# szcompressor/SZ3

Measured on AMD Instinct MI355X. Metric: compression throughput GB/s + ratio at fixed abs errBound, 512^3 f32, higher is better.
Workload: dtype f32; 1 GPU; C2: 3D float32 512x512x512 synthetic field per GPU, Lorenzo predictor, abs errBound=0.001, device-resident in -> device-resident Huffman payload; parallelism=slab1, algo=HIP_LORENZO(16), exchange=none (one rank)

## Files before the change

include/sz3hip.h:

```cpp
#ifndef SZ3HIP_H
#define SZ3HIP_H
#include <stddef.h>
#include <stdint.h>

#ifdef __cplusplus
extern "C" {
#endif

#define SZ3HIP_FLOAT 0
#define SZ3HIP_DOUBLE 1
#define SZ3HIP_UINT8 2
#define SZ3HIP_INT8 3
#define SZ3HIP_UINT16 4
#define SZ3HIP_INT16 5
#define SZ3HIP_UINT32 6
#define SZ3HIP_INT32 7
#define SZ3HIP_UINT64 8
#define SZ3HIP_INT64 9

enum { SZ3HIP_EB_ABS = 0, SZ3HIP_EB_REL, SZ3HIP_EB_PSNR, SZ3HIP_EB_L2NORM, SZ3HIP_EB_ABS_AND_REL, SZ3HIP_EB_ABS_OR_REL };

enum {
    SZ3HIP_ALGO_LORENZO_REG = 0,
    SZ3HIP_ALGO_INTERP_LORENZO = 1,
// ... 51 lines not shown
size_t sz3hip_compress_blob(sz3hip_config *conf, int dataType, const void *data, char *blob, size_t cap);
int sz3hip_decompress_blob(const sz3hip_config *conf, int dataType, const char *blob, size_t size, void *decData);
int sz3hip_peek_config(sz3hip_config *conf, const char *cmpData, size_t cmpSize);

typedef struct sz3hip_ctx sz3hip_ctx;

sz3hip_ctx *sz3hip_ctx_create(int device, uint64_t max_elems, int dataType);
void sz3hip_ctx_destroy(sz3hip_ctx *ctx);
size_t sz3hip_payload_bound(const sz3hip_ctx *ctx, uint64_t n);
size_t sz3hip_payload_bound_max(const sz3hip_ctx *ctx, uint64_t n);
size_t sz3hip_payload_bound_conf(const sz3hip_ctx *ctx, const sz3hip_config *conf, int worst_case);

int sz3hip_minmax_device(sz3hip_ctx *ctx, const void *d_in, uint64_t n, double *min_out, double *max_out, void *stream);

int sz3hip_compress_stage1(sz3hip_ctx *ctx, const sz3hip_config *conf, const void *d_in, void *stream);
void *sz3hip_histogram_ptr(sz3hip_ctx *ctx);
size_t sz3hip_histogram_len(const sz3hip_ctx *ctx);
int sz3hip_ctx_set_histogram(sz3hip_ctx *ctx, void *d_hist);
int sz3hip_compress_stage2(sz3hip_ctx *ctx, void *d_payload, size_t cap, void *stream);
int sz3hip_compress_finish(sz3hip_ctx *ctx, size_t *payload_size, void *stream);
int sz3hip_compress_device(sz3hip_ctx *ctx, const sz3hip_config *conf, const void *d_in, void *d_payload, size_t cap,
                           size_t *payload_size, void *stream);
int sz3hip_decompress_device(sz3hip_ctx *ctx, const void *d_payload, size_t payload_size, void *d_out, void *stream);

typedef struct sz3hip_stats {
    uint64_t n, n_value_outliers, n_delta_outliers, n_chunks, bitstream_bytes, payload_bytes;
    uint32_t n_symbols, max_code_len;
    uint32_t narrow_codes;
    uint32_t reserved;
} sz3hip_stats;
int sz3hip_get_stats(sz3hip_ctx *ctx, sz3hip_stats *st);

typedef struct sz3hip_tuner_report {
    int32_t ran;
    int32_t use_interp;
    uint64_t sample_block_size, n_filtered, n_blocks;
    int32_t profiling;
    int32_t interpAlgo, interpDirection;
    int32_t speculated;
    double interpAlpha, interpBeta;
    double est_bytes[8];
} sz3hip_tuner_report;
int sz3hip_get_tuner_report(sz3hip_ctx *ctx, sz3hip_tuner_report *rep);

void sz3hip_set_profiling(sz3hip_ctx *ctx, int on);
int sz3hip_get_stage_times(sz3hip_ctx *ctx, const char **names, float *ms, int max);
void sz3hip_ctx_forget(sz3hip_ctx *ctx);
void sz3hip_ctx_set_speculation(sz3hip_ctx *ctx, int off);
void sz3hip_ctx_set_deterministic(sz3hip_ctx *ctx, int on);
void sz3hip_ctx_set_tuner_exact(sz3hip_ctx *ctx, int on);
void sz3hip_get_spec_stats(const sz3hip_ctx *ctx, uint32_t *hits, uint32_t *misses);
int sz3hip_last_call_fused(const sz3hip_ctx *ctx);
int sz3hip_last_call_q16(const sz3hip_ctx *ctx);
void sz3hip_ctx_set_fused(sz3hip_ctx *ctx, int on);
int sz3hip_lab_build(void);
int sz3hip_debug_copy_codes(sz3hip_ctx *ctx, uint16_t *host_codes, uint64_t n);
int sz3hip_debug_decode_info(sz3hip_ctx *ctx, uint32_t *out4);
void sz3hip_debug_force_generic(int on);
void sz3hip_debug_flags(int flags);

typedef struct sz3hip_comm sz3hip_comm;
#define SZ3HIP_COMM_ID_BYTES 128
sz3hip_comm *sz3hip_comm_create_local(int ndev, const int *devices);
int sz3hip_comm_unique_id(unsigned char *id128);
sz3hip_comm *sz3hip_comm_create_rank(int nranks, int rank, int device, const unsigned char *id128);
void sz3hip_comm_destroy(sz3hip_comm *comm);
int sz3hip_comm_size(const sz3hip_comm *comm);
int sz3hip_comm_rank(const sz3hip_comm *comm);
int sz3hip_comm_local_size(const sz3hip_comm *comm);
int sz3hip_comm_device(const sz3hip_comm *comm, int member);
int sz3hip_comm_allreduce_histogram(sz3hip_comm *comm, sz3hip_ctx *const *ctxs, void *const *streams);
int sz3hip_comm_allreduce_u64(sz3hip_comm *comm, void *const *d_bufs, size_t count, void *const *streams);
int sz3hip_comm_allreduce_minmax(sz3hip_comm *comm, double *mins, double *maxs, void *const *streams);


size_t sz3hip_compress_rank(sz3hip_comm *comm, const sz3hip_config *global_conf, int dataType, const void *slab_data,
                            char *blob, size_t cap, sz3hip_config *slab_conf);
size_t sz3hip_assemble_container(const sz3hip_config *global_conf, int dataType, int G, const sz3hip_config *slab_confs,
                                 const char *const *blobs, const size_t *blob_sizes, char *out, size_t cap);

#ifdef __cplusplus
}
#endif
#endif
```

sz3_amd/__init__.py:

```python
import ctypes as C
import os

import numpy as np

_HERE = os.path.dirname(os.path.abspath(__file__))
LIB_PATH = os.environ.get("SZ3HIP_LIB") or os.path.join(_HERE, "libsz3hip.so")

EB_ABS, EB_REL, EB_PSNR, EB_L2NORM, EB_ABS_AND_REL, EB_ABS_OR_REL = range(6)
ALGO_LORENZO_REG, ALGO_INTERP_LORENZO, ALGO_INTERP, ALGO_NOPRED, ALGO_LOSSLESS = range(5)
ALGO_HIP_LORENZO = 16
ALGO_HIP_INTERP = 17
INTERP_ALGO_LINEAR, INTERP_ALGO_CUBIC = 0, 1
SZ_FLOAT, SZ_DOUBLE = 0, 1


class SZ3HipError(RuntimeError):
    def __init__(self, code, msg):
        super().__init__("sz3hip error %d: %s" % (code, msg))
        self.code = code


class _CConfig(C.Structure):
    _fields_ = [
        ("N", C.c_int32), ("dims", C.c_uint64 * 4), ("num", C.c_uint64),
        ("cmprAlgo", C.c_uint8), ("errorBoundMode", C.c_uint8),
        ("absErrorBound", C.c_double), ("relErrorBound", C.c_double),
        ("psnrErrorBound", C.c_double), ("l2normErrorBound", C.c_double),
        ("openmp", C.c_uint8), ("quantbinCnt", C.c_int32), ("blockSize", C.c_int32),
        ("predDim", C.c_uint8), ("dataType", C.c_uint8),
        ("lorenzo", C.c_uint8), ("lorenzo2", C.c_uint8), ("regression", C.c_uint8), ("regression2", C.c_uint8),
        ("interpAlgo", C.c_uint8), ("interpDirection", C.c_uint8),
        ("interpAnchorStride", C.c_int32), ("interpAlpha", C.c_double), ("interpBeta", C.c_double),
    ]


class _CTunerReport(C.Structure):
    _fields_ = [("ran", C.c_int32), ("use_interp", C.c_int32), ("sample_block_size", C.c_uint64), ("n_filtered", C.c_uint64),
                ("n_blocks", C.c_uint64), ("profiling", C.c_int32), ("interpAlgo", C.c_int32), ("interpDirection", C.c_int32),
                ("speculated", C.c_int32), ("interpAlpha", C.c_double), ("interpBeta", C.c_double), ("est_bytes", C.c_double * 8)]


class _CStats(C.Structure):
    _fields_ = [("n", C.c_uint64), ("n_value_outliers", C.c_uint64), ("n_delta_outliers", C.c_uint64),
                ("n_chunks", C.c_uint64), ("bitstream_bytes", C.c_uint64), ("payload_bytes", C.c_uint64),
                ("n_symbols", C.c_uint32), ("max_code_len", C.c_uint32),
                ("narrow_codes", C.c_uint32), ("reserved", C.c_uint32)]


_lib = None


def _share_torch_hip_runtime():
    try:
        import importlib.util
        import sys
        if "torch" in sys.modules:
            return
        if os.environ.get("SZ3HIP_TORCH_PRELOAD", "0") == "1":
# ... 56 lines not shown
    L.sz3hip_compress.argtypes = [P(_CConfig), C.c_int, C.c_void_p, C.c_void_p, C.c_size_t]
    L.sz3hip_decompress.restype = C.c_int
    L.sz3hip_decompress.argtypes = [P(_CConfig), C.c_int, C.c_void_p, C.c_size_t, C.c_void_p]
    L.sz3hip_peek_config.restype = C.c_int
    L.sz3hip_compress_from_device.restype = C.c_size_t
    L.sz3hip_compress_from_device.argtypes = [P(_CConfig), C.c_int, C.c_void_p, P(C.c_int64), C.c_void_p, C.c_size_t, C.c_void_p]
    L.sz3hip_decompress_to_device.restype = C.c_int
    L.sz3hip_decompress_to_device.argtypes = [P(_CConfig), C.c_int, C.c_void_p, C.c_size_t, C.c_void_p, P(C.c_int64), C.c_void_p]
    L.sz3hip_peek_config.argtypes = [P(_CConfig), C.c_void_p, C.c_size_t]
    L.sz3hip_ctx_create.restype = C.c_void_p
    L.sz3hip_ctx_create.argtypes = [C.c_int, C.c_uint64, C.c_int]
    L.sz3hip_ctx_destroy.argtypes = [C.c_void_p]
    L.sz3hip_payload_bound.restype = C.c_size_t
    L.sz3hip_payload_bound.argtypes = [C.c_void_p, C.c_uint64]
    L.sz3hip_payload_bound_max.restype = C.c_size_t
    L.sz3hip_payload_bound_max.argtypes = [C.c_void_p, C.c_uint64]
    L.sz3hip_minmax_device.restype = C.c_int
    L.sz3hip_minmax_device.argtypes = [C.c_void_p, C.c_void_p, C.c_uint64, P(C.c_double), P(C.c_double), C.c_void_p]
    L.sz3hip_compress_stage1.restype = C.c_int
    L.sz3hip_compress_stage1.argtypes = [C.c_void_p, P(_CConfig), C.c_void_p, C.c_void_p]
    L.sz3hip_histogram_ptr.restype = C.c_void_p
    L.sz3hip_histogram_ptr.argtypes = [C.c_void_p]
    L.sz3hip_histogram_len.restype = C.c_size_t
    L.sz3hip_histogram_len.argtypes = [C.c_void_p]
    L.sz3hip_ctx_set_histogram.restype = C.c_int
    L.sz3hip_ctx_set_histogram.argtypes = [C.c_void_p, C.c_void_p]
    L.sz3hip_compress_stage2.restype = C.c_int
    L.sz3hip_compress_stage2.argtypes = [C.c_void_p, C.c_void_p, C.c_size_t, C.c_void_p]
    L.sz3hip_compress_finish.restype = C.c_int
    L.sz3hip_compress_finish.argtypes = [C.c_void_p, P(C.c_size_t), C.c_void_p]
    L.sz3hip_compress_device.restype = C.c_int
    L.sz3hip_compress_device.argtypes = [C.c_void_p, P(_CConfig), C.c_void_p, C.c_void_p, C.c_size_t, P(C.c_size_t), C.c_void_p]
    L.sz3hip_decompress_device.restype = C.c_int
    L.sz3hip_decompress_device.argtypes = [C.c_void_p, C.c_void_p, C.c_size_t, C.c_void_p, C.c_void_p]
    L.sz3hip_get_stats.restype = C.c_int
    L.sz3hip_get_stats.argtypes = [C.c_void_p, P(_CStats)]
    L.sz3hip_get_tuner_report.restype = C.c_int
    L.sz3hip_get_tuner_report.argtypes = [C.c_void_p, P(_CTunerReport)]
    L.sz3hip_set_profiling.argtypes = [C.c_void_p, C.c_int]
    L.sz3hip_ctx_forget.argtypes = [C.c_void_p]
    L.sz3hip_ctx_forget.restype = None
    L.sz3hip_ctx_set_speculation.argtypes = [C.c_void_p, C.c_int]
    L.sz3hip_ctx_set_speculation.restype = None
    L.sz3hip_ctx_set_deterministic.argtypes = [C.c_void_p, C.c_int]
    L.sz3hip_ctx_set_deterministic.restype = None
    L.sz3hip_ctx_set_tuner_exact.argtypes = [C.c_void_p, C.c_int]
    L.sz3hip_ctx_set_tuner_exact.restype = None
    L.sz3hip_set_stock_format.argtypes = [C.c_int]
    L.sz3hip_set_stock_format.restype = None
    L.sz3hip_last_call_fused.argtypes = [C.c_void_p]
    L.sz3hip_last_call_fused.restype = C.c_int
    L.sz3hip_last_call_q16.argtypes = [C.c_void_p]
    L.sz3hip_last_call_q16.restype = C.c_int
    L.sz3hip_ctx_set_fused.argtypes = [C.c_void_p, C.c_int]
    L.sz3hip_ctx_set_fused.restype = None
    L.sz3hip_get_spec_stats.argtypes = [C.c_void_p, C.POINTER(C.c_uint32), C.POINTER(C.c_uint32)]
    L.sz3hip_get_spec_stats.restype = None
    L.sz3hip_payload_bound_conf.restype = C.c_size_t
    L.sz3hip_payload_bound_conf.argtypes = [C.c_void_p, C.c_void_p, C.c_int]
    L.sz3hip_get_stage_times.restype = C.c_int
    L.sz3hip_get_stage_times.argtypes = [C.c_void_p, P(C.c_char_p), P(C.c_float), C.c_int]
    L.sz3hip_debug_copy_codes.restype = C.c_int
    L.sz3hip_debug_copy_codes.argtypes = [C.c_void_p, C.c_void_p, C.c_uint64]
    L.sz3hip_debug_force_generic.argtypes = [C.c_int]
    L.sz3hip_config_load_n.restype = C.c_size_t
    L.sz3hip_config_load_n.argtypes = [P(_CConfig), C.c_void_p, C.c_size_t]
    L.sz3hip_comm_create_local.restype = C.c_void_p
    L.sz3hip_comm_create_local.argtypes = [C.c_int, P(C.c_int)]
    L.sz3hip_comm_unique_id.restype = C.c_int
    L.sz3hip_comm_unique_id.argtypes = [C.c_void_p]
    L.sz3hip_comm_create_rank.restype = C.c_void_p
    L.sz3hip_comm_create_rank.argtypes = [C.c_int, C.c_int, C.c_int, C.c_void_p]
    L.sz3hip_comm_destroy.argtypes = [C.c_void_p]
    for f in ("size", "rank", "local_size"):
        getattr(L, "sz3hip_comm_" + f).restype = C.c_int
        getattr(L, "sz3hip_comm_" + f).argtypes = [C.c_void_p]
    L.sz3hip_comm_device.restype = C.c_int
    L.sz3hip_comm_device.argtypes = [C.c_void_p, C.c_int]
    L.sz3hip_comm_allreduce_histogram.restype = C.c_int
    L.sz3hip_comm_allreduce_histogram.argtypes = [C.c_void_p, P(C.c_void_p), P(C.c_void_p)]
    L.sz3hip_comm_allreduce_u64.restype = C.c_int
    L.sz3hip_comm_allreduce_u64.argtypes = [C.c_void_p, P(C.c_void_p), C.c_size_t, P(C.c_void_p)]
    L.sz3hip_comm_allreduce_minmax.restype = C.c_int
    L.sz3hip_comm_allreduce_minmax.argtypes = [C.c_void_p, P(C.c_double), P(C.c_double), P(C.c_void_p)]
    L.sz3hip_compress_rank.restype = C.c_size_t
    L.sz3hip_compress_rank.argtypes = [C.c_void_p, P(_CConfig), C.c_int, C.c_void_p, C.c_void_p, C.c_size_t, P(_CConfig)]
    L.sz3hip_assemble_container.restype = C.c_size_t
    L.sz3hip_assemble_container.argtypes = [P(_CConfig), C.c_int, C.c_int, P(_CConfig), P(C.c_void_p), P(C.c_size_t), C.c_void_p, C.c_size_t]
    L.SZ_compress_args.restype = C.c_void_p
    L.SZ_compress_args.argtypes = [C.c_int, C.c_void_p, P(C.c_size_t), C.c_int, C.c_double, C.c_double, C.c_double,
                                   C.c_size_t, C.c_size_t, C.c_size_t, C.c_size_t, C.c_size_t]
    L.SZ_decompress.restype = C.c_void_p
    L.SZ_decompress.argtypes = [C.c_int, C.c_void_p, C.c_size_t, C.c_size_t, C.c_size_t, C.c_size_t, C.c_size_t, C.c_size_t]
    L.free_buf.argtypes = [C.c_void_p]
    _lib = L
    return L


def _check(rc):
    if rc != 0:
        raise SZ3HipError(rc, lib().sz3hip_last_error().decode())


_SZ_TYPES = {"float32": 0, "float64": 1, "uint8": 2, "int8": 3, "uint16": 4, "int16": 5, "uint32": 6, "int32": 7, "uint64": 8, "int64": 9}


# ... 221 lines not shown

    def finish(self, stream=0):
        sz = C.c_size_t()
        _check(lib().sz3hip_compress_finish(self._h, C.byref(sz), stream))
        return int(sz.value)

    def compress(self, conf, d_in, d_payload, cap, stream=0):
        sz = C.c_size_t()
        _check(lib().sz3hip_compress_device(self._h, C.byref(conf._c), d_in, d_payload, int(cap), C.byref(sz), stream))
        return int(sz.value)

    def decompress(self, d_payload, size, d_out, stream=0):
        _check(lib().sz3hip_decompress_device(self._h, d_payload, int(size), d_out, stream))

    def stats(self):
        st = _CStats()
        lib().sz3hip_get_stats(self._h, C.byref(st))
        return {k: int(getattr(st, k)) for k, _ in _CStats._fields_}

    def tuner_report(self):
        r = _CTunerReport()
        lib().sz3hip_get_tuner_report(self._h, C.byref(r))
        out = {k: getattr(r, k) for k, _ in _CTunerReport._fields_ if k not in ("est_bytes", "speculated")}
        out["est_bytes"] = [float(x) for x in r.est_bytes]
        self.speculated = int(r.speculated)
        return out

    def set_profiling(self, on=True):
        lib().sz3hip_set_profiling(self._h, int(on))

    def forget(self):
        lib().sz3hip_ctx_forget(self._h)

    def set_speculation(self, on=True, backoff=True):
        lib().sz3hip_ctx_set_speculation(self._h, (0 if backoff else 2) if on else 1)

    def set_deterministic(self, on=True):
        lib().sz3hip_ctx_set_deterministic(self._h, int(on))

    def set_tuner_exact(self, on=True):
        lib().sz3hip_ctx_set_tuner_exact(self._h, int(on))

    def set_fused(self, on=True):
        lib().sz3hip_ctx_set_fused(self._h, int(on))

    @property
    def fused(self):
        return bool(lib().sz3hip_last_call_fused(self._h))

    @property
    def q16(self):
        return bool(lib().sz3hip_last_call_q16(self._h))

    def spec_stats(self):
        h, m = C.c_uint32(), C.c_uint32()
        lib().sz3hip_get_spec_stats(self._h, C.byref(h), C.byref(m))
        return int(h.value), int(m.value)

    def payload_bound_conf(self, conf, worst_case=False):
        return int(lib().sz3hip_payload_bound_conf(self._h, C.byref(conf._c), int(bool(worst_case))))

    def stage_times(self):
        names = (C.c_char_p * 16)()
        ms = (C.c_float * 16)()
        k = lib().sz3hip_get_stage_times(self._h, names, ms, 16)
        return {names[i].decode(): float(ms[i]) for i in range(k)}

    def debug_codes(self, n):
        out = np.empty(int(n), dtype=np.uint16)
        _check(lib().sz3hip_debug_copy_codes(self._h, out.ctypes.data, int(n)))
        return out


COMM_ID_BYTES = 128


class Comm:

    def __init__(self, handle):
        if not handle:
            raise SZ3HipError(lib().sz3hip_last_error_code(), lib().sz3hip_last_error().decode())
        self._h = handle

    @staticmethod
    def unique_id():
        buf = (C.c_ubyte * COMM_ID_BYTES)()
        _check(lib().sz3hip_comm_unique_id(buf))
        return bytes(buf)

    @classmethod
    def local(cls, ndev=0, devices=None):
        arr = (C.c_int * len(devices))(*devices) if devices else None
        return cls(lib().sz3hip_comm_create_local(int(ndev if not devices else len(devices)), arr))

    @classmethod
    def rank(cls, nranks, rank, device, id_bytes):
        b = (C.c_ubyte * COMM_ID_BYTES).from_buffer_copy(bytes(id_bytes))
        return cls(lib().sz3hip_comm_create_rank(int(nranks), int(rank), int(device), b))

    def close(self):
        if self._h:
            lib().sz3hip_comm_destroy(self._h)
            self._h = None

    @property
    def size(self):
# ... 60 lines not shown
```

sz3_amd/csrc/sz3hip_api.cpp:

```cpp
#include <hip/hip_runtime.h>

#include <dlfcn.h>
#include <math.h>
#include <stdarg.h>
#include <stdio.h>
#include <stdlib.h>
#include <string.h>

#include <sched.h>
#include <unistd.h>
#include <algorithm>
#include <atomic>
#include <chrono>
#include <mutex>
#include <string>
#include <thread>
#include <vector>

#include "../../include/sz3c.h"
#include "../../include/sz3hip.h"
#include "sz3hip_format.h"
#include "sz3hip_internal.h"
#include "sz3hip_stock_geom.h"
#include "sz3hip_kernels.h"
// ... 504 lines not shown
    hh.eb = eb;
    hh.n = num;
    hh.chunk_syms = SZH_CHUNK_SYMS;
    hh.n_chunks = (num + SZH_CHUNK_SYMS - 1) / SZH_CHUNK_SYMS;
    hh.interp_alpha = ip.alpha;
    hh.interp_beta = ip.beta;
    hh.interp_id = (uint32_t)ip.interp_id;
    hh.interp_dir = (uint32_t)ip.direction;
    hh.anchor_stride = ip.anchor_stride;
    ctx->stage1_done = true;
    ctx->stage2_done = false;
    return 0;
}

static bool book_spec_ok(const sz3hip_ctx *ctx, uint32_t predictor, uint32_t radius) {
    return ctx->book_idx >= 0 && ctx->spec_off != 1 && (ctx->spec_skip == 0 || ctx->spec_off == 2) && !(szk_dbg_flags & 131072) &&
           ctx->book_pred == predictor && ctx->book_radius == radius;
}
static int lorenzo_k1(sz3hip_ctx *ctx, int N, const uint64_t *dims, const void *d_in, double eb, int radius, uint64_t num,
                      uint64_t out_cap, bool allow_narrow, szk_k1_params &p, hipStream_t s) {
    memset(&p, 0, sizeof(p));
    for (int i = 0; i < 4; i++) p.d[i] = 1;
    for (int i = 0; i < N; i++) p.d[4 - N + i] = dims[i];
    p.lat = szk_make_lattice(eb);
    p.radius = (uint32_t)radius;
    p.out_cap = out_cap;
    p.hist = ctx->d_hist;
    p.hist_partial = ctx->d_hist_partial;
    p.n_vout = ctx->d_counters + 0;
    p.n_dout = ctx->d_counters + 1;
    p.vout_idx = ctx->d_vout_idx;
    p.dout_idx = ctx->d_dout_idx;
    p.vout_val = ctx->d_vout_val;
    p.dout_val = ctx->d_dout_val;
    p.mode.probe_big = reinterpret_cast<uint32_t *>(ctx->d_counters + 4);
    p.mode.n_total = num;
    p.mode.n_samples = (num / SZK_PROBE_STRIDE) * 64 + std::min<uint64_t>(64, num % SZK_PROBE_STRIDE);
    p.mode.allow = allow_narrow && radius >= 128;
    p.mode.pack_wide = allow_narrow ? (uint32_t)ctx->pack_wide : 0u;
    p.wide16 = ctx->wide16 < 0 ? (ctx->dtype == SZ3HIP_DOUBLE ? 1u : 0u) : (uint32_t)ctx->wide16;
    p.range = reinterpret_cast<uint32_t *>(ctx->d_counters + 8);
    p.hint_narrow = allow_narrow ? ctx->narrow_hint : -1;
    if ((ctx->hist_exposed || ctx->hist_reduced) && p.hint_narrow > 0) p.hint_narrow = -1;
    p.hint_q16 = allow_narrow && ctx->dtype == SZ3HIP_FLOAT && ctx->q16_hint > 0 && ctx->q16_block == 0 ? 1 : 0;
    p.q16_flag = reinterpret_cast<uint32_t *>(ctx->d_counters + 11) + 1;
    const bool samp = allow_narrow && radius >= 128 && N <= 3 && p.d[3] % 256 == 0 && num >= SZK_SAMP_MIN_ELEMS && !ctx->hist_exposed && !ctx->hist_reduced &&
                      !(szk_dbg_flags & 65536);
    if (samp) {
        const int fresh = ctx->book_idx < 0 ? 0 : 1 - ctx->book_idx;
        p.samp.words = reinterpret_cast<uint32_t *>(ctx->d_counters + 16);
        p.samp.enc = ctx->bk[fresh].enc;
        p.samp.lens = ctx->bk[fresh].lens;
        p.samp.info = ctx->bk[fresh].info;
        p.seg_bits = ctx->d_seg_bits;
        p.seg_made = reinterpret_cast<uint32_t *>(ctx->d_counters + 10) + 1;
    }
    if (!samp && allow_narrow && book_spec_ok(ctx, 0, (uint32_t)radius) && ctx->cb_hint == 0 && !ctx->lists_long && !ctx->hist_exposed) {
        p.spec_lens = ctx->bk[ctx->book_idx].lens;
        p.seg_bits = ctx->d_seg_bits;
        p.seg_made = reinterpret_cast<uint32_t *>(ctx->d_counters + 10) + 1;
        p.defer_fold = ctx->hist_exposed || ctx->hist_reduced || (szk_dbg_flags & 16777216) ? 0 : 1;
        const uint64_t need = szk_fuse_scratch_words(N, p.d);
        if (need && ctx->fuse_on && !ctx->hist_reduced && (!ctx->spec_exact || ctx->last_spec_hit)) {
            p.fuse_slots = reinterpret_cast<uint32_t *>(ctx->d_codes);
            p.fuse_cap_words = (ctx->max_n + 64) / 2;
            if (need > p.fuse_cap_words && need <= 2 * num + (1u << 18)) {
                if (ctx->fuse_scratch_words < need) {
                    if (ctx->d_fuse_scratch) (void)hipFree(ctx->d_fuse_scratch);
                    ctx->d_fuse_scratch = nullptr;
                    ctx->fuse_scratch_words = 0;
                    if (hipMalloc((void **)&ctx->d_fuse_scratch, need * 4) == hipSuccess) ctx->fuse_scratch_words = need;
                    else (void)hipGetLastError();
                }
                if (ctx->fuse_scratch_words >= need) {
                    p.fuse_slots = ctx->d_fuse_scratch;
                    p.fuse_cap_words = ctx->fuse_scratch_words;
                }
            }
            p.fuse = 1;
            p.fuse_enc = ctx->bk[ctx->book_idx].enc;
            p.fuse_info = ctx->bk[ctx->book_idx].info;
            p.seg_base = ctx->d_seg_base;
            p.fuse_flag = reinterpret_cast<uint32_t *>(ctx->d_counters + 11);
        }
    }
    p.prof_ev0 = p.prof_ev1 = nullptr;
    if (ctx->profiling && allow_narrow) {
        p.prof_ev0 = ctx->ev[ST_K1_KERNEL][0];
        p.prof_ev1 = ctx->ev[ST_K1_KERNEL][1];
        ctx->ev_used[ST_K1_KERNEL] = true;
    }
    return szk_launch_k1(ctx->dtype, N, d_in, ctx->d_codes, &p, s);
}
static int stage1_lorenzo(sz3hip_ctx *ctx, const sz3hip_config *conf, const void *d_in, double eb, int radius, uint64_t num, hipStream_t s) {
    szk_k1_params p;
    prof_begin(ctx, ST_K1, s);
    int rc = lorenzo_k1(ctx, conf->N, conf->dims, d_in, eb, radius, num, ctx->cur_out_cap, true, p, s);
    ctx->mode = p.mode;
    ctx->range_ready = p.range_kept != 0;
    ctx->s1_assumed_narrow = p.assumed_narrow != 0;
    ctx->s1_q16 = p.assumed_q16 != 0;
    ctx->s1_spec = p.spec_lens != nullptr;
    ctx->seg_expected = p.seg_expected != 0 && !(szk_dbg_flags & 33554432);
    ctx->fold_rows = p.defer_fold ? p.fold_rows : 0;
    ctx->fold_range = p.range;
    ctx->s1_fused = p.fused != 0;
// ... 1003 lines not shown
        if (ctx->range_ready && !cb.range_ready)
            HIPCHK(hipMemsetAsync(ctx->d_counters + 8, 0, 16, s));
        prof_begin(ctx, ST_CODEBOOK, s);
        int rcb = szk_launch_codebook(ctx->d_hist, &cb, s);
        prof_end(ctx, ST_CODEBOOK, s);
        if (rcb) return fail(SZ3HIP_EHIP, "codebook kernel launch failed (%d)", rcb);
    }
    szk_layout_params lp;
    lp.proto = ctx->proto;
    lp.n_vout = ctx->d_counters + 0;
    lp.n_dout = ctx->d_counters + 1;
    lp.out_cap = ctx->cur_out_cap;
    lp.info = ctx->bk[used].info;
    lp.state = ctx->d_state;
    lp.side_bytes = ctx->proto.predictor == 2 ? ctx->d_blk_counters + 2 : nullptr;
    szk_asm_params ap;
    memset(&ap, 0, sizeof(ap));
    ap.n_vout = ctx->d_counters + 0;
    ap.n_dout = ctx->d_counters + 1;
    ap.out_cap = ctx->cur_out_cap;
    ap.t_is_32bit = ap.q_is_32bit = ctx->dtype == SZ3HIP_FLOAT;
    ap.state = ctx->d_state;
    ap.payload = (uint8_t *)d_payload;
    ap.cap = cap;
    ap.total_words = ctx->d_counters + 2;
    ap.lens = ctx->bk[used].lens;
    ap.chunk_words = ctx->d_chunk_words;
    ap.sub_bits = ctx->d_sub_bits;
    ap.vout_idx = ctx->d_vout_idx;
    ap.dout_idx = ctx->d_dout_idx;
    ap.vout_val = ctx->d_vout_val;
    ap.dout_val = ctx->d_dout_val;
    ap.side = ctx->proto.predictor == 2 ? ctx->d_blk_side : nullptr;
    ap.assumed_narrow = ctx->s1_assumed_narrow ? 1 : 0;
    ap.q16_flag = ctx->s1_q16 && ctx->proto.predictor == 0 ? reinterpret_cast<const uint32_t *>(ctx->d_counters + 11) + 1 : nullptr;
    ap.mode = ctx->mode;
    ap.samp_words = samp_words;
    szk_merge_args mg;
    memset(&mg, 0, sizeof(mg));
    const bool merge = fused && ctx->s1_fused && ctx->seg_expected;
    if (ctx->s1_fused && !merge) return fail(SZ3HIP_EHIP, "internal: fused stage 1 without the merging encoder");
    if (merge) {
        mg.slots = ctx->s1_slots;
        mg.seg_base = ctx->d_seg_base;
        mg.fuse_flag = reinterpret_cast<const uint32_t *>(ctx->d_counters + 11);
    }
    prof_begin(ctx, ST_ENCODE, s);
    int rc = szk_launch_encode(ctx->d_codes, n, ctx->bk[used].enc, ctx->bk[used].info, (int)ctx->proto.radius, ctx->mode, ctx->d_chunk_words,
                               ctx->d_chunk_off, ctx->d_counters + 2, ctx->d_state, (uint8_t *)d_payload, &lp, &ap, s,
                               (fused || (samp_words && ctx->s1_samp_in)) && ctx->seg_expected ? ctx->d_seg_bits : nullptr, reinterpret_cast<uint32_t *>(ctx->d_counters + 10) + 1,
                               (fused || wide || how == S2_SAMPLED) ? &er : nullptr, merge ? &mg : nullptr);
    prof_end(ctx, ST_ENCODE, s);
    if (rc) return fail(SZ3HIP_EHIP, "encode kernel launch failed (%d)", rc);
    if (wide) {
        HIPCHK(hipStreamWaitEvent(s, ctx->ev_book, 0));
        if (szk_launch_book_verdict(ctx->bk[fresh].info, ctx->bk[fresh].lens, ctx->bk[used].info, ctx->bk[used].lens,
                                    reinterpret_cast<const uint32_t *>(ctx->d_counters + 7), reinterpret_cast<const uint32_t *>(ctx->d_counters + 8),
                                    ctx->d_state, ctx->d_hist, ctx->spec_exact, s))
            return fail(SZ3HIP_EHIP, "verdict kernel launch failed");
    }
    prof_end(ctx, ST_SPAN, s);
    ctx->pub_zero = ctx->d_hist == ctx->d_hist_own && !ctx->hist_exposed && !(szk_dbg_flags & 268435456);
    ctx->pub_seq++;
    ctx->pub_blk_zero = ctx->pub_zero && ctx->d_blk_counters && ctx->d_blk_stats5;
    if (szk_launch_publish(ctx->d_state, ctx->h_state, ctx->h_pub_seq, ctx->pub_seq, ctx->pub_zero ? (void *)ctx->d_hist : nullptr,
                           SZH_HIST_BINS * 8 + SZ_COUNTER_BYTES, s, ctx->blk_spec ? blk_sel_count(ctx) : nullptr,
                           ctx->pub_blk_zero ? (void *)ctx->d_blk_counters : nullptr, ctx->pub_blk_zero ? ctx->d_blk_stats5 : nullptr))
        return fail(SZ3HIP_EHIP, "publish kernel launch failed");
    ctx->pub_stream = s;
    return 0;
}

static int wait_published(sz3hip_ctx *ctx) {
    volatile uint32_t *seq = ctx->h_pub_seq;
    for (uint64_t it = 1;; it++) {
        if (*seq == ctx->pub_seq) break;
        if ((it & 0xFFFF) == 0) {
            const hipError_t q = hipStreamQuery(ctx->pub_stream);
            if (q == hipSuccess) {
                if (*seq == ctx->pub_seq) break;
                return fail(SZ3HIP_EHIP, "stage 2 finished without publishing its state");
            }
            if (q != hipErrorNotReady) return fail(SZ3HIP_EHIP, "HIP error while waiting for stage 2: %s", hipGetErrorString(q));
        }
        if (it < 4096) __builtin_ia32_pause();
        else if (it < 65536) sched_yield();
        else usleep(20);
    }
    __atomic_thread_fence(__ATOMIC_ACQUIRE);
    return 0;
}
extern "C" int sz3hip_compress_finish(sz3hip_ctx *ctx, size_t *payload_size, void *stream) {
    hipStream_t s = (hipStream_t)stream;
    HIPCHK(hipSetDevice(ctx->device));
    if (!ctx->stage2_done) return fail(SZ3HIP_EINVAL, "finish called before stage2");
    if (int rw = wait_published(ctx)) return rw;
    bool blk_miss = false;
    if (ctx->blk_spec) {
        const uint64_t others = ctx->h_state->blk_others;
        const bool all = (ctx->blk_spec_mask & 1u) && (others << BLK_EXIT_SHIFT) < ctx->blk_spec_nblocks;
        ctx->blk_others = others;
        blk_miss = all != ctx->blk_spec_all;
        ctx->blk_spec = false;
        if (blk_miss) ctx->blk_dec_valid = false;
    }
    const bool fused_miss = (ctx->s1_fused && (ctx->h_state->miss_kind != 0 || ctx->h_state->mispredict != 0)) || blk_miss;
// ... 7 lines not shown
        if (ctx->h_state->miss_kind & 128u) {
            ctx->q16_hint = 0;
            ctx->q16_block = 16;
        }
        if (ctx->h_state->mispredict || (ctx->h_state->miss_kind & 2u)) ctx->cb_hint = ctx->cb_part = -1;
        const int spec_was = ctx->spec_off;
        ctx->spec_off = 1;
        sz3hip_config conf = ctx->s1_conf;
        int rc1 = sz3hip_compress_stage1(ctx, &conf, ctx->s1_in, stream);
        ctx->spec_off = spec_was;
        if (rc1) return rc1;
        rc1 = stage2_launch(ctx, ctx->s2_payload, ctx->s2_cap, s, S2_CLASSIC);
        if (rc1) return rc1;
        if (int rw = wait_published(ctx)) return rw;
        ctx->spec_penalty = ctx->spec_penalty ? std::min(8, 2 * ctx->spec_penalty) : 1;
        ctx->spec_skip = ctx->spec_penalty;
    } else if (ctx->s2_spec) {
        if (ctx->h_state->miss_kind) {
            ctx->spec_misses++;
            const uint32_t kind = ctx->h_state->miss_kind;
            const bool redo_book = (kind & (2u | 4u)) != 0;
            if (redo_book) {
                if (kind & 2u) ctx->cb_hint = ctx->cb_part = -1;
                HIPCHK(hipMemsetAsync(ctx->d_counters + 7, 0, 24, s));
                ctx->range_ready = false;
            }
            int rc2 = stage2_launch(ctx, ctx->s2_payload, ctx->s2_cap, s, redo_book ? S2_CLASSIC : S2_REENCODE);
            if (rc2) return rc2;
            if (int rw = wait_published(ctx)) return rw;
            ctx->spec_penalty = ctx->spec_penalty ? std::min(8, 2 * ctx->spec_penalty) : 1;
            ctx->spec_skip = ctx->spec_penalty;
        } else {
            ctx->spec_hits++;
            ctx->spec_penalty = 0;
        }
    } else if (ctx->s2_samp && ctx->h_state->miss_kind) {
        HIPCHK(hipMemsetAsync(ctx->d_counters + 7, 0, 24, s));
        ctx->range_ready = false;
        int rc2 = stage2_launch(ctx, ctx->s2_payload, ctx->s2_cap, s, S2_CLASSIC);
        if (rc2) return rc2;
        if (int rw = wait_published(ctx)) return rw;
    } else if (ctx->spec_skip > 0) {
        ctx->spec_skip--;
    }
    if (ctx->h_state->mispredict) {
        ctx->cb_hint = ctx->cb_part = -1;
        HIPCHK(hipMemsetAsync(ctx->d_counters + 7, 0, 24, s));
        ctx->range_ready = false;
        int rc2 = stage2_launch(ctx, ctx->s2_payload, ctx->s2_cap, s, S2_CLASSIC);
        if (rc2) return rc2;
        if (int rw = wait_published(ctx)) return rw;
        if (ctx->h_state->mispredict) return fail(SZ3HIP_EHIP, "code book was not built (both forms declined)");
    }
    ctx->stage1_done = ctx->stage2_done = false;
    if (ctx->pub_zero && ctx->h_state->miss_kind == 0 && ctx->h_state->mispredict == 0) {
        ctx->pre_cleared = true;
        ctx->pre_stream = ctx->pub_stream;
        ctx->blk_pre_cleared = ctx->pub_blk_zero;
        ctx->blk_pre_stream = ctx->pub_stream;
    } else if (ctx->d_hist == ctx->d_hist_own && !ctx->hist_exposed && !(szk_dbg_flags & 268435456)) {
        if (hipMemsetAsync(ctx->d_hist, 0, SZH_HIST_BINS * 8 + SZ_COUNTER_BYTES, s) == hipSuccess) {
            ctx->pre_cleared = true;
            ctx->pre_stream = s;
        }
    }
    const szk_state &st = *ctx->h_state;
    if (st.hdr.magic != SZH_MAGIC) return fail(SZ3HIP_EHIP, "device did not produce a payload header (kernel fault?)");
    if (st.hdr.n_vout > 32768 || st.hdr.n_dout > 32768) {
        uint8_t *pl = (uint8_t *)ctx->s2_payload;
        const int tb = st.hdr.dtype == SZ3HIP_FLOAT ? 4 : 8;
        int rs = 0;
        if (st.hdr.n_vout > 32768) rs |= szk_sort_list_pairs((uint64_t *)(pl + st.off.vout_idx), pl + st.off.vout_val, st.hdr.n_vout, tb, s);
        if (st.hdr.n_dout > 32768) rs |= szk_sort_list_pairs((uint64_t *)(pl + st.off.dout_idx), pl + st.off.dout_val, st.hdr.n_dout, (int)st.hdr.qbytes, s);
        if (rs) return fail(SZ3HIP_EHIP, "sorting the payload's outlier lists failed");
    }
    ctx->book_idx = ctx->book_pending;
    ctx->book_pred = st.hdr.predictor;
    ctx->book_radius = st.hdr.radius;
    ctx->lists_long = st.hdr.n_vout > 2048 || st.hdr.n_dout > 2048;
    ctx->cb_hint = st.n_symbols > SZK_CB_SMALL_SYMS ? 1 : 0;
    ctx->cb_part = szk_cb_part(st.n_symbols, st.hdr.sym_count);
    if (st.hdr.predictor == 2) ctx->blk_wide = st.hdr.sym_count > 3000 ? 1 : 0;
    ctx->stats.n = st.hdr.n;
    ctx->stats.n_value_outliers = st.hdr.n_vout;
    ctx->stats.n_delta_outliers = st.hdr.n_dout;
    ctx->stats.n_chunks = st.hdr.n_chunks;
    ctx->stats.bitstream_bytes = st.hdr.bitstream_words * 4;
    ctx->stats.payload_bytes = st.hdr.payload_bytes;
    ctx->stats.max_code_len = st.hdr.max_len;
    ctx->stats.n_symbols = st.n_symbols;
    ctx->stats.narrow_codes = ctx->mode.allow && (uint64_t)st.probe[0] * 4096ull <= ctx->mode.n_samples;
    if (st.hdr.predictor == 0 && ctx->mode.allow) ctx->narrow_hint = ctx->stats.narrow_codes ? 1 : 0;
    if (st.hdr.predictor == 0 && ctx->mode.allow) {
        if (ctx->q16_block > 0) ctx->q16_block--;
        ctx->q16_hint = ctx->stats.narrow_codes && st.probe[3] == 0 ? 1 : 0;
    }
    ctx->stats.reserved = (ctx->wide16 > 0 ? 1u : 0u) | (st.probe[1] << 1);
    if (st.hdr.predictor == 1)
    {
        const bool was_big = ctx->hist_big > 0;
        ctx->hist_big = (uint64_t)st.probe[4] * 100ull > st.hdr.n ? 1 : 0;
        ctx->hist_tail = was_big && ctx->hist_big && st.probe[5] > (1u << 18) ? 1 : (was_big ? 0 : ctx->hist_tail);
    }
    if (st.hdr.predictor == 0 && ctx->mode.allow && ctx->mode.n_samples) {
        ctx->wide16 = (uint64_t)st.probe[1] * 300ull > ctx->mode.n_samples ? 1 : 0;
        ctx->pack_wide = (uint64_t)st.probe[2] * 50ull > ctx->mode.n_samples ? 1 : 0;
// ... 113 lines not shown
    out->N = h.ndim;
    for (int i = 0; i < h.ndim; i++) out->dims[i] = h.dims[4 - h.ndim + i];
    out->interp_id = (int)h.interp_id;
    out->direction = (int)h.interp_dir;
    out->anchor_stride = h.anchor_stride;
    out->alpha = h.interp_alpha;
    out->beta = h.interp_beta;
    out->eb = h.eb;
    out->radius = (int)h.radius;
    *n_unpred = nv;
    return 0;
}
int szi_stock_export(sz3hip_ctx *ctx, const szg_geom *g, const uint64_t *d_blk_base, uint16_t *d_em, void *d_unpred, uint64_t n_unpred,
                     uint32_t *d_tile_cnt, uint64_t *d_tile_base, void *stream) {
    hipStream_t s = (hipStream_t)stream;
    HIPCHK(hipSetDevice(ctx->device));
    if (szk_launch_stock_from_elem(ctx->dtype, g, d_blk_base, ctx->d_codes, ctx->d_vout_idx, ctx->d_vout_val, n_unpred, d_tile_cnt, d_tile_base, d_em, d_unpred, s))
        return fail(SZ3HIP_EHIP, "stock export kernels failed");
    ctx->stage1_done = ctx->stage2_done = false;
    return 0;
}
int szi_stock_import(sz3hip_ctx *ctx, const szi_stock_params *p, const szg_geom *g, const uint64_t *d_blk_base, const uint16_t *d_em,
                     const void *d_unpred, uint64_t n_unpred, uint32_t *d_tile_cnt, uint64_t *d_tile_base, uint64_t *d_vout_idx, void *d_vout_val,
                     uint32_t *d_bad, void *d_out, void *stream) {
    hipStream_t s = (hipStream_t)stream;
    HIPCHK(hipSetDevice(ctx->device));
    uint64_t num = 1;
    for (int i = 0; i < p->N; i++) num *= p->dims[i];
    if (num > ctx->max_n) return fail(SZ3HIP_EINVAL, "array exceeds the context capacity");
    HIPCHK(hipMemsetAsync(d_bad, 0, 4, s));
    if (szk_launch_stock_to_elem(ctx->dtype, g, d_blk_base, d_em, d_unpred, n_unpred, d_tile_cnt, d_tile_base, ctx->d_codes, d_vout_idx, d_vout_val, d_bad, s))
        return fail(SZ3HIP_EHIP, "stock import kernels failed");
    szk_interp_params ip;
    memset(&ip, 0, sizeof(ip));
    ip.N = p->N;
    for (int i = 0; i < p->N; i++) ip.dims[i] = p->dims[i];
    ip.interp_id = p->interp_id;
    ip.direction = p->direction;
    ip.anchor_stride = p->anchor_stride;
    ip.alpha = p->alpha;
    ip.beta = p->beta;
    ip.eb = p->eb;
    ip.radius = p->radius;
    if (szk_launch_interp_decompress(ctx->dtype, &ip, nullptr, (uint64_t)(uintptr_t)d_vout_idx, (uint64_t)(uintptr_t)d_vout_val, n_unpred, ctx->d_codes, d_out, s))
        return fail(SZ3HIP_EHIP, "interpolation decoder launch failed");
    uint32_t bad = 0;
    HIPCHK(hipMemcpyAsync(&bad, d_bad, 4, hipMemcpyDeviceToHost, s));
    HIPCHK(hipStreamSynchronize(s));
    if (bad) return fail(SZ3HIP_EFORMAT, "corrupt stock stream: its codes and its list of unpredictable values do not fit together");
    return 0;
}
extern "C" int sz3hip_last_call_fused(const sz3hip_ctx *ctx) { return ctx->last_fused ? 1 : 0; }
extern "C" int sz3hip_last_call_q16(const sz3hip_ctx *ctx) { return ctx->last_q16 ? 1 : 0; }
extern "C" int sz3hip_lab_build(void) {
#ifdef SZ3HIP_LAB
    return 1;
#else
    return 0;
#endif
}
extern "C" void sz3hip_ctx_set_fused(sz3hip_ctx *ctx, int on) { ctx->fuse_on = on != 0 && sz3hip_lab_build(); }
extern "C" void sz3hip_get_spec_stats(const sz3hip_ctx *ctx, uint32_t *hits, uint32_t *misses) {
    *hits = ctx->spec_hits;
    *misses = ctx->spec_misses;
}
extern "C" void sz3hip_debug_flags(int flags) {
    szk_dbg_flags = flags;
    szk_interp_novec = (flags & 128) != 0;
    szk_interp_min_blocks = (flags & 4194304) ? 1 : 256;
}
extern "C" int sz3hip_debug_codebook_info(sz3hip_ctx *ctx, uint64_t *out16) {
    HIPCHK(hipSetDevice(ctx->device));
    HIPCHK(hipDeviceSynchronize());
    szk_cb_info info;
    HIPCHK(hipMemcpy(&info, ctx->bk[ctx->book_idx < 0 ? 0 : ctx->book_idx].info, sizeof(info), hipMemcpyDeviceToHost));
    out16[0] = info.n_symbols; out16[1] = info.max_len; out16[2] = info.sym_min; out16[3] = info.sym_count;
    for (int i = 0; i < 12; i++) out16[4 + i] = info.ts[i];
    return 0;
}

extern "C" int sz3hip_debug_decode_info(sz3hip_ctx *ctx, uint32_t *out4) {
    out4[0] = ctx->last_half;
    out4[1] = ctx->last_carry;
    out4[2] = (uint32_t)ctx->half_skip;
    out4[3] = 0;
    return 0;
}

extern "C" int sz3hip_decompress_device(sz3hip_ctx *ctx, const void *d_payload, size_t payload_size, void *d_out,
                                        void *stream) {
    hipStream_t s = (hipStream_t)stream;
    HIPCHK(hipSetDevice(ctx->device));
    ctx->blk_pre_cleared = false;
    if (payload_size < sizeof(szh_header)) return fail(SZ3HIP_EFORMAT, "payload shorter than its header");
    szh_header h;
    uint32_t *ovf = reinterpret_cast<uint32_t *>(ctx->d_counters + 12);
    if (!ctx->h_ovf) {
        HIPCHK(hipHostMalloc((void **)&ctx->h_ovf, 8));
        *ctx->h_ovf = 0;
        HIPCHK(hipMemsetAsync(ovf, 0, 4, s));
    }
    HIPCHK(hipMemcpyAsync(&ctx->h_state->hdr, d_payload, sizeof(szh_header), hipMemcpyDeviceToHost, s));
    HIPCHK(hipMemcpyAsync(ctx->h_ovf, ovf, 4, hipMemcpyDeviceToHost, s));
    HIPCHK(hipStreamSynchronize(s));
    if (*ctx->h_ovf) ctx->half_skip = 8;
    else if (ctx->half_skip > 0) ctx->half_skip--;
// ... 176 lines not shown
```

sz3_amd/csrc/sz3hip_internal.h:

```cpp
#ifndef SZ3HIP_INTERNAL_H
#define SZ3HIP_INTERNAL_H
#include <hip/hip_runtime.h>
#include <string.h>

#include "../../include/sz3hip.h"
#include "sz3hip_format.h"
#include "sz3hip_kernels.h"

int szi_fail(int code, const char *fmt, ...) __attribute__((format(printf, 2, 3)));
struct sz3hip_ctx;
struct szg_geom;
struct szi_stock_params {
    int N;
    uint64_t dims[4];
    int interp_id, direction;
    uint64_t anchor_stride;
    double alpha, beta, eb;
    int radius;
};
int szi_stock_stage1_outcome(sz3hip_ctx *ctx, szi_stock_params *out, uint64_t *n_unpred, void *stream);
int szi_stock_export(sz3hip_ctx *ctx, const szg_geom *g, const uint64_t *d_blk_base, uint16_t *d_em, void *d_unpred, uint64_t n_unpred,
                     uint32_t *d_tile_cnt, uint64_t *d_tile_base, void *stream);
int szi_stock_import(sz3hip_ctx *ctx, const szi_stock_params *p, const szg_geom *g, const uint64_t *d_blk_base, const uint16_t *d_em,
                     const void *d_unpred, uint64_t n_unpred, uint32_t *d_tile_cnt, uint64_t *d_tile_base, uint64_t *d_vout_idx, void *d_vout_val,
                     uint32_t *d_bad, void *d_out, void *stream);
int szi_stage1_with_larger_lists(sz3hip_ctx *ctx, const sz3hip_config *conf, const void *d_in, uint64_t need, void *stream, bool any_number = false);
int szi_pretune_host(sz3hip_ctx *ctx, const sz3hip_config *conf, const void *h_in);
void szi_pretune_cancel(sz3hip_ctx *ctx);
void szi_ctx_exact_default(sz3hip_ctx *ctx, int on);
int szi_tuner_took_lorenzo(sz3hip_ctx *ctx, int *quantbinCnt);
void szi_run_parallel(int n, const std::function<void(int)> &f);
size_t szi_zstd_size(const void *src, size_t n);
void *szi_histogram_for_exchange(sz3hip_ctx *ctx);
void szi_exchange_call(sz3hip_ctx *ctx, bool on);

struct Writer {
    unsigned char *p;
    template <class V> void put(V v) {
        memcpy(p, &v, sizeof(V));
        p += sizeof(V);
    }
};
struct Reader {
    const unsigned char *p;
    template <class V> V get() {
        V v;
        memcpy(&v, p, sizeof(V));
        p += sizeof(V);
        return v;
    }
};

enum { ST_K1 = 0, ST_CODEBOOK, ST_ENCODE, ST_ASSEMBLE, ST_DEC_HUFF, ST_DEC_RECON, ST_TUNER, ST_K1_KERNEL, ST_SPAN, ST_COUNT };

struct sz3hip_ctx {
    int device;
    int dtype;
    uint64_t max_n, out_cap, cur_out_cap, max_chunks;
    uint64_t out_alloc;
    uint64_t force_out_cap;
    uint16_t *d_codes;
    uint64_t *d_hist;
    uint64_t *d_hist_own;
    uint64_t *d_counters;
    uint32_t *d_hist_partial;
    void *d_dense2;
    size_t dense2_elems;
    void *d_work;
    int narrow_hint;
    int cb_hint;
    int cb_part;
    int q16_hint;
    int q16_block;
    bool s1_q16;
    bool last_q16;
    bool range_ready;
    bool hist_exposed;
    int half_skip;
    uint32_t *h_ovf;
    void *s2_payload;
    size_t s2_cap;
    struct Book {
        uint32_t *enc;
        uint8_t *lens;
        szk_cb_info *info;
    } bk[2];
    int book_idx, book_pending;
    uint32_t book_pred, book_radius;
    bool s2_spec;
    bool lists_long;
    int spec_off;
    int spec_exact;
    int spec_skip, spec_penalty;
    uint32_t spec_hits, spec_misses;
    hipEvent_t ev_done;
    uint32_t *h_pub_seq;
    uint32_t pub_seq;
    bool pub_zero;
    hipStream_t pub_stream;
    hipStream_t pre_stream;
    bool pre_cleared;
    bool s1_assumed_narrow;
    sz3hip_config s1_conf;
    const void *s1_in;
    uint32_t redo_calls;
    bool s1_spec;
    bool seg_expected;
    uint32_t fold_rows;
    uint32_t *fold_range;
    uint16_t *d_seg_bits;
    uint32_t *d_seg_base;
    uint32_t *d_fuse_scratch;
    uint64_t fuse_scratch_words;
    const uint32_t *s1_slots;
    bool fuse_on;
    bool s1_fused;
    bool s1_samp;
    bool s1_samp_in;
    bool s2_samp;
    bool last_fused;
    bool last_spec_hit;
    int blk_wide;
    uint64_t blk_cap;
    uint8_t *d_blk_sel;
    int64_t *d_blk_coef;
    uint32_t *d_blk_rank, *d_blk_comp;
    uint8_t *d_blk_side;
    uint64_t *d_blk_counters;
// ... 91 lines not shown
```

sz3_amd/csrc/sz3hip_kernels.h:

```cpp
#ifndef SZ3HIP_KERNELS_H
#define SZ3HIP_KERNELS_H
#include <hip/hip_runtime.h>
#include <stdint.h>
#include "sz3hip_format.h"

struct szk_lattice {
    double recip, two_eb, eb;
    float recip_f, two_eb_f, eb_lo_f;
};
static inline szk_lattice szk_make_lattice(double eb) {
    szk_lattice l;
    l.eb = eb;
    l.two_eb = 2.0 * eb;
    l.recip = 1.0 / l.two_eb;
    l.recip_f = (float)l.recip;
    l.two_eb_f = (float)l.two_eb;
    float e = (float)eb;
    if ((double)e > eb) e = __builtin_nextafterf(e, 0.0f);
    l.eb_lo_f = e;
    return l;
}

#define SZK_K1_GRID 2048u

#define SZK_PROBE_STRIDE 32768ull
struct szk_mode {
    uint32_t *probe_big;
    uint32_t pack_wide;
    uint64_t n_samples;
    uint64_t n_total;
    uint32_t allow;
};

struct szk_cb_info;
#define SZK_SAMP_UNITS 1024u
#define SZK_SAMP_ROLES 128u
#define SZK_SAMP_MIN_ELEMS (1ull << 22)
#define SZK_SAMP_SEEN_LEN 16u
#define SZK_SAMP_WORDS 512u
#define SZK_SAMP_TICKET 320u
#define SZK_SAMP_LENS 384u
#define SZK_SAMP_READY 448u
struct szk_samp {
    uint32_t *words;
    uint32_t *enc;
    uint8_t *lens;
    szk_cb_info *info;
};
struct szk_k1_params {
    uint64_t d[4];
    szk_lattice lat;
    uint32_t radius;
    uint32_t dbg;
    szk_mode mode;
    uint64_t out_cap;
    uint64_t *hist;
    uint32_t *hist_partial;
    uint64_t *n_vout, *n_dout;
    uint64_t *vout_idx, *dout_idx;
    void *vout_val, *dout_val;
    void *prof_ev0, *prof_ev1;
    uint32_t wide16;
    uint32_t *range;
    int hint_narrow;
    const uint8_t *spec_lens;
    uint16_t *seg_bits;
    uint32_t *seg_made;
    int seg_expected;
    int assumed_narrow;
    int hint_q16;
    int assumed_q16;
    uint32_t *q16_flag;
    int defer_fold;
    uint32_t fold_rows;
    int range_kept;
    int fuse;
    int fused;
    const uint32_t *fuse_enc;
    const szk_cb_info *fuse_info;
    uint32_t *fuse_slots;
    uint64_t fuse_cap_words;
    uint32_t *seg_base;
    uint32_t *fuse_flag;
    uint32_t fuse_geom[4];
    szk_samp samp;
    int samp_in_launch;
};

struct szk_cb_info {
    uint32_t n_symbols, max_len, sym_min, sym_count;
    uint32_t win_lo, reserved;
    uint32_t esc_sym, pad0;
    uint64_t ts[12];
    uint32_t first_code[SZH_MAX_LEN + 2];
};
struct szk_cb_params {
    uint32_t *enc;
    uint8_t *lens;
    uint64_t *keys;
    uint16_t *syms;
// ... 169 lines not shown
    uint64_t *n_vout, *vout_idx;
    void *vout_val;
    uint64_t out_cap;
    uint32_t hist_big;
    uint32_t hist_tail;
    uint32_t *far_cnt;
    void *dense2;
    uint64_t dense2_elems;
};
struct szk_interp_pass {
    int N, dir, interp_id, old_api, subpass, radius;
    int kind;
    int no_store;
    uint64_t dims[4], off[4], start[4], step[4], cnt[4];
    uint64_t total, s, bsz;
    uint64_t batch_stride;
    double eb, eb_recip;
    uint64_t *n_vout, *vout_idx;
    void *vout_val;
    uint64_t out_cap;
};
extern int szk_interp_novec;
extern int szk_interp_min_blocks;
int szk_interp_levels_ok(const szk_interp_params *ip);
int szk_launch_interp_compress(int dtype, const szk_interp_params *ip, const void *d_in, void *d_work, uint16_t *codes,
                               uint64_t *hist, hipStream_t s);
int szk_launch_interp_decompress(int dtype, const szk_interp_params *ip, const uint8_t *payload, uint64_t vout_idx_off,
                                 uint64_t vout_val_off, uint64_t n_vout, uint16_t *codes, void *d_out, hipStream_t s);

int szk_launch_profile_blocks(int dtype, const void *d_in, int N, const uint64_t *dims, uint64_t bs, uint64_t stride, double abseb,
                              uint8_t *d_flags, uint64_t *total_out, hipStream_t s);
int szk_launch_gather_blocks(int dtype, const void *d_in, int N, const uint64_t *dims, uint64_t edge, const uint64_t *d_starts,
                             uint32_t nblocks, void *d_out, hipStream_t s);
#define SZK_TRIAL_MAX_PASSES 64
int szk_launch_interp_trials(int dtype, const szk_interp_params *ips, uint32_t ntrials, const void *d_samples, void *d_work,
                             uint16_t *codes, uint32_t nblocks, uint64_t *d_hists, szk_interp_pass *h_passes, szk_interp_pass *d_passes,
                             uint32_t *h_np, uint32_t *d_np, int keep_codes, hipStream_t s);
int szk_launch_code_cost(const uint64_t *hist, const uint64_t *counters, uint64_t *d_res, uint32_t n_books, uint64_t total,
                         int unpred_is_code0, hipStream_t s);

struct szk_view {
    uint64_t dims[4];
    int64_t str[4];
    int contig;
};
int szk_launch_gather(int sz_type , int widen, const void *d_in, const szk_view *v, void *d_out, uint32_t *d_flag, hipStream_t s);
int szk_launch_scatter(int sz_type, int narrow, const void *d_in, void *d_out, const szk_view *v, hipStream_t s);
int szk_launch_int_to_f64(int sz_type , const void *d_in, uint64_t n, double *d_out, uint32_t *d_flag, hipStream_t s);
int szk_launch_f64_to_int(int sz_type, const double *d_in, uint64_t n, void *d_out, hipStream_t s);
int szk_launch_hist_add(uint64_t *d_dst, const uint64_t *d_src, uint32_t n, hipStream_t s);
int szk_launch_minmax(int dtype, const void *d_in, uint64_t n, double *d_partial , double *d_out , hipStream_t s);
int szk_launch_k1(int dtype, int ndim, const void *d_in, uint16_t *codes, szk_k1_params *p, hipStream_t s);
int szk_launch_codebook(const uint64_t *d_hist, const szk_cb_params *p, hipStream_t s);
int szk_launch_encode(const uint16_t *codes, uint64_t n, const uint32_t *d_enc, const szk_cb_info *info, int radius,
                      szk_mode mode, uint16_t *chunk_words, uint64_t *group_off , uint64_t *total_words,
                      const szk_state *state, uint8_t *payload, const szk_layout_params *layout,
                      const szk_asm_params *asmp , hipStream_t s,
                      const uint16_t *seg_bits = nullptr ,
                      const uint32_t *seg_made = nullptr ,
                      const szk_encode_roles *roles = nullptr,
                      const szk_merge_args *merge = nullptr );
int szk_launch_book_verdict(const szk_cb_info *fresh, const uint8_t *fresh_lens, const szk_cb_info *used, const uint8_t *used_lens,
                            const uint32_t *mispredict, const uint32_t *range, szk_state *state,
                            const uint64_t *hist , int exact , hipStream_t s);
struct szg_geom;
int szk_launch_stock_to_elem(int dtype, const szg_geom *g, const uint64_t *d_blk_base, const uint16_t *d_em, const void *d_unpred, uint64_t n_unpred,
                             uint32_t *d_tile_cnt, uint64_t *d_tile_base, uint16_t *d_codes, uint64_t *d_vout_idx, void *d_vout_val, uint32_t *d_bad,
                             hipStream_t s);
int szk_launch_stock_from_elem(int dtype, const szg_geom *g, const uint64_t *d_blk_base, const uint16_t *d_codes, const uint64_t *d_vout_idx,
                               const void *d_vout_val, uint64_t n_vout, uint32_t *d_tile_cnt, uint64_t *d_tile_base, uint16_t *d_em, void *d_unpred,
                               hipStream_t s);
int szk_launch_stock_ranks(const szg_geom *g, const uint64_t *d_blk_base, uint64_t *d_rank, hipStream_t s);
int szk_launch_stock_huff_encode(const uint16_t *d_em, uint64_t n, const uint8_t *d_clen, const uint64_t *d_cbits, uint32_t *d_tile_bits, uint64_t *d_tile_base,
                                 uint32_t *d_out_words, uint64_t out_words_cap, uint64_t *total_bits, hipStream_t s);
struct szk_stock_tree_dev {
    const uint32_t *L, *R;
    const int32_t *C;
    const uint8_t *t;
    const uint32_t *lut;
    uint32_t nc;
    int32_t offset;
};
int szk_launch_stock_huff_decode(const szk_stock_tree_dev *tr, const uint32_t *d_words, uint64_t nbytes, uint64_t n, uint64_t *d_start, uint64_t *d_last,
                                 uint64_t *d_next, uint64_t *d_base, uint32_t *d_count, uint32_t *d_flags, uint16_t *d_em, int *passes, hipStream_t s);
struct szk_slr_params {
    uint64_t d[3];
    uint32_t nb[3];
    uint32_t B, N;
    double eb;
    uint32_t radius;
    const uint16_t *codes;
    const uint8_t *kind;
    const void *coef;
    const void *unpred;
    uint64_t n_unpred;
    const uint64_t *tile_base;
    void *out;
    uint32_t *bad;
    uint64_t dw;
    uint32_t nbw;
};
int szk_launch_stock_lorenzo_reg(int dtype, const szk_slr_params *p, uint64_t n, uint32_t *d_tile_cnt, uint64_t *d_tile_base, hipStream_t s);
struct szk_slw_params {
    uint64_t d[3];
    uint32_t nb[3];
    uint32_t B, N;
// ... 54 lines not shown
```

sz3_amd/csrc/sz3hip_kernels.hip:

```cpp
#include <hip/hip_runtime.h>
#include <cstddef>
#include <stdint.h>
#include <type_traits>
#include <mutex>
#include <utility>
#include <vector>
#include "sz3hip_format.h"
#include "sz3hip_kernels.h"

#include "sz3hip_devutil.h"

template <typename T>
__global__ __launch_bounds__(256) void k_minmax(const T *__restrict__ in, uint64_t n, double *partial) {
    double mn = INFINITY, mx = -INFINITY;
    bool has_nan = false;
    for (uint64_t i = (uint64_t)blockIdx.x * blockDim.x + threadIdx.x; i < n; i += (uint64_t)gridDim.x * blockDim.x) {
        double v = (double)in[i];
        if (v < mn) mn = v;
        if (v > mx) mx = v;
        has_nan |= (v != v);
    }
    (void)has_nan;
#pragma unroll
    for (int d = WAVE / 2; d > 0; d >>= 1) {
// ... 850 lines not shown
            p.vout_idx[pos] = c.oq_idx[k];
            if (sizeof(T) == 4) reinterpret_cast<uint32_t *>(p.vout_val)[pos] = (uint32_t)c.oq_val[k];
            else reinterpret_cast<uint64_t *>(p.vout_val)[pos] = c.oq_val[k];
        }
    }
    c.oq_n = 0;
}
template <typename T>
__device__ __forceinline__ void narrow_rare(NarrowCtx<T> &c, uint64_t gi, const typename QTraits<T>::UQ (&delta)[4], uint32_t tmask, uint32_t badmask) {
    using Q = typename QTraits<T>::Q;
    using OQV = typename NarrowCtx<T>::OQV;
    const szk_k1_params &p = *c.p;
    constexpr uint32_t OQ = MarchLds<1, false>::OQ;
    {
        unsigned long long pd = wave_append_run((uint32_t)__popc(tmask & 15u), p.n_dout);
#pragma unroll
        for (int i = 0; i < 4; i++)
            if ((tmask >> i) & 1u) {
                if (pd < p.out_cap) {
                    p.dout_idx[pd] = gi + i;
                    ((Q *)p.dout_val)[pd] = (Q)delta[i];
                }
                pd++;
            }
    }
#pragma unroll
    for (int i = 0; i < 4; i++) {
        const bool is_vout = (badmask >> i) & 1u;
        const unsigned long long vm = __ballot(is_vout);
        if (vm) {
            c.oq_n = (uint32_t)__builtin_amdgcn_readfirstlane((int)c.oq_n);
            if (c.oq_n + WAVE > OQ) narrow_oq_flush(c);
            if (is_vout) {
                const uint32_t slot = c.oq_n + (uint32_t)__popcll(vm & ((1ull << c.lane) - 1ull));
                c.oq_idx[slot] = gi + i;
                const T raw = c.in[gi + i];
                OQV bits = 0;
                memcpy(&bits, &raw, sizeof(T));
                c.oq_val[slot] = bits;
            }
            c.oq_n += (uint32_t)__popcll(vm);
        }
    }
    {
        const uint32_t cnt = (uint32_t)__popc(tmask & 15u);
        const unsigned long long b0 = __ballot(cnt & 1u), b1 = __ballot(cnt & 2u), b2 = __ballot(cnt & 4u), any = b0 | b1 | b2;
        if (any && c.lane == __ffsll((long long)any) - 1)
            hist_add_ranged(p.hist, p.range, 0u, (unsigned long long)(__popcll(b0) + 2 * __popcll(b1) + 4 * __popcll(b2)));
    }
}
template <typename T> __device__ __forceinline__ bool samp_take(const T *__restrict__ in, const szk_lattice &latp, uint32_t d0, uint32_t d1, uint32_t d2, uint32_t *words, uint32_t role, uint32_t *s_h);
__device__ __forceinline__ void samp_book(const szk_samp &sp, uint32_t radius, uint8_t *pool);
#define SAMP_POOL_BYTES (SZK_CB_SMALL_SYMS * 28 + 256)
template <typename T, typename PUT>
__device__ __forceinline__ bool samp_poll(NarrowCtx<T> &c, bool spin, PUT put) {
    volatile uint32_t *s_have = c.s_have;
    const uint32_t wv = (uint32_t)__builtin_amdgcn_readfirstlane((int)(threadIdx.x / WAVE));
    if (wv != 0) {
        uint32_t h = (uint32_t)__builtin_amdgcn_readfirstlane((int)*s_have);
        if (!h) {
            if (!spin) return false;
            do {
                __builtin_amdgcn_s_sleep(16);
                h = (uint32_t)__builtin_amdgcn_readfirstlane((int)*s_have);
            } while (!h);
        }
        __builtin_amdgcn_fence(__ATOMIC_ACQUIRE, "workgroup");
        c.have_len = 1;
        return true;
    }
    uint32_t r = __hip_atomic_load(const_cast<uint32_t *>(c.samp_words) + SZK_SAMP_READY, __ATOMIC_RELAXED, __HIP_MEMORY_SCOPE_AGENT);
    r = (uint32_t)__builtin_amdgcn_readfirstlane((int)r);
    if (!r) {
        if (!spin) return false;
        do {
            __builtin_amdgcn_s_sleep(32);
            r = __hip_atomic_load(const_cast<uint32_t *>(c.samp_words) + SZK_SAMP_READY, __ATOMIC_RELAXED, __HIP_MEMORY_SCOPE_AGENT);
            r = (uint32_t)__builtin_amdgcn_readfirstlane((int)r);
        } while (!r);
    }
    const uint32_t w = __hip_atomic_load(const_cast<uint32_t *>(c.samp_words) + SZK_SAMP_LENS + c.lane, __ATOMIC_RELAXED, __HIP_MEMORY_SCOPE_AGENT);
#pragma unroll
    for (int j = 0; j < 4; j++) put(4u * (uint32_t)c.lane + j, (w >> (8 * j)) & 0xFFu);
    __builtin_amdgcn_fence(__ATOMIC_RELEASE, "workgroup");
    __builtin_amdgcn_wave_barrier();
    if (c.lane == 0) *s_have = 1u;
    c.have_len = 1;
    return true;
}
template <typename T, int NW, int TY> struct NarrowPlane {
    Quad<T> rq[NW][TY + 1];
    T rl[NW][TY + 1];
    bool rok[NW][TY + 1];
};
template <typename T>
__device__ __forceinline__ void fuse_sweep(NarrowCtx<T> &c, uint32_t nw) {
    uint32_t *out = c.slot + c.slot_w;
    auto sweep = [&](uint32_t i) {
        const uint2 wv = *reinterpret_cast<const uint2 *>(&c.stage[i]);
        *reinterpret_cast<uint2 *>(&c.stage[i]) = make_uint2(0u, 0u);
#if defined(LAB_FUSE) && (LAB_FUSE & 32)
        *reinterpret_cast<unsigned long long *>(&out[i]) = (unsigned long long)wv.x | ((unsigned long long)wv.y << 32);
#else
        __builtin_nontemporal_store((unsigned long long)wv.x | ((unsigned long long)wv.y << 32), reinterpret_cast<unsigned long long *>(&out[i]));
#endif
    };
    const uint32_t i0 = 2u * (uint32_t)c.lane;
    if (i0 < nw) sweep(i0);
    if (i0 + 2u * WAVE < nw) sweep(i0 + 2u * WAVE);
    if (nw > 4u * WAVE)
        for (uint32_t i = i0 + 4u * WAVE; i < nw; i += 2u * WAVE) sweep(i);
}
template <typename T>
__device__ __forceinline__ void fuse_flush_lines(NarrowCtx<T> &c) {
#if defined(LAB_FUSE) && (LAB_FUSE & 4)
    const uint32_t nfl = 0;
    c.st_cnt &= 31u;
#else
    const uint32_t nfl = c.st_cnt & ~31u;
#endif
    if (nfl == 0) return;
    fuse_sweep(c, nfl);
    const uint32_t left = c.st_cnt - nfl;
    if (left) {
// ... 425 lines not shown
        if constexpr (FUSE) {
            c.slot_base = task * p.fuse_geom[3];
            c.slot = p.fuse_slots + c.slot_base;
            c.slot_w = 0;
        }
        if (x0 + MARCH_TX <= c.d0 && y0 + TY <= c.d1) narrow_task<T, NDIM, TY, false, FUSE, SAMP>(c, lat, x0, y0, z0, w);
        else narrow_task<T, NDIM, TY, true, FUSE, SAMP>(c, lat, x0, y0, z0, w);
        if constexpr (FUSE) {
            c.st_cnt = (uint32_t)__builtin_amdgcn_readfirstlane((int)c.st_cnt);
            if (c.st_cnt) {
                fuse_sweep(c, (c.st_cnt + 1u) & ~1u);
                c.st_cnt = 0;
                __builtin_amdgcn_wave_barrier();
            }
        }
    }
    narrow_oq_flush(c);
    if (SAMP) return;
    __syncthreads();
    uint32_t *row = p.hist_partial + (uint64_t)blockIdx.x * HIST_WIN;
    for (int bnn = threadIdx.x; bnn < HIST_WIN; bnn += 256) {
        const int t = bnn - (HIST_WIN / 2 - 127);
        row[bnn] = (t >= 0 && t < 255) ? lh[t * 4] + lh[t * 4 + 1] + lh[t * 4 + 2] + lh[t * 4 + 3] : 0u;
    }
}

#define Q16_LIM 4095.0f
typedef float v2f32 __attribute__((ext_vector_type(2)));
typedef unsigned short v2u16 __attribute__((ext_vector_type(2)));
__device__ __forceinline__ uint32_t pk_sub16(uint32_t a, uint32_t b) {
    return __builtin_bit_cast(uint32_t, (v2u16)(__builtin_bit_cast(v2u16, a) - __builtin_bit_cast(v2u16, b)));
}
__device__ __forceinline__ uint32_t pk_add16(uint32_t a, uint32_t b) {
    return __builtin_bit_cast(uint32_t, (v2u16)(__builtin_bit_cast(v2u16, a) + __builtin_bit_cast(v2u16, b)));
}
__device__ __forceinline__ uint32_t pk_min16(uint32_t a, uint32_t b) {
    return __builtin_bit_cast(uint32_t, __builtin_elementwise_min(__builtin_bit_cast(v2u16, a), __builtin_bit_cast(v2u16, b)));
}
__device__ __forceinline__ uint32_t pk_max16(uint32_t a, uint32_t b) {
    return __builtin_bit_cast(uint32_t, __builtin_elementwise_max(__builtin_bit_cast(v2u16, a), __builtin_bit_cast(v2u16, b)));
}
__device__ __forceinline__ uint32_t pk_lo16(uint32_t a, uint32_t b) { return __builtin_amdgcn_perm(b, a, 0x05040100u); }
__device__ __forceinline__ uint32_t mad16_lo(uint32_t p, uint32_t add) {
    uint32_t d;
    asm("v_mad_u32_u16 %0, %1, 16, %2" : "=v"(d) : "v"(p), "v"(add));
    return d;
}
__device__ __forceinline__ uint32_t mad16_hi(uint32_t p, uint32_t add) {
    uint32_t d;
    asm("v_mad_u32_u16 %0, %1, 16, %2 op_sel:[1,0,0,0]" : "=v"(d) : "v"(p), "v"(add));
    return d;
}
#define Q16_LEN_OFF (NARROW_BINS * 16)
template <int TY> struct Q16Plane {
    float4 rq[TY + 1];
    float rl[TY + 1];
    bool rok[TY + 1];
};
template <int TY, bool EDGE, bool SAMP>
__device__ __forceinline__ void narrow16_task(NarrowCtx<float> &c, const Lattice<float> &lat, uint32_t *q16_flag, uint32_t x0, uint32_t y0, uint32_t z0) {
    const uint32_t d0 = c.d0, d1 = c.d1, d2 = c.d2;
    const int lane = c.lane;
    const uint32_t x = x0 + 4u * (uint32_t)lane;
    const bool xok = EDGE ? x < d0 : true;
    const uint32_t lane_off = xok ? x : 0u;
    const bool has_left = x0 > 0;
    const uint32_t c4 = ((uint32_t)lane & 3u) * 4u;
    uint8_t *const lds = reinterpret_cast<uint8_t *>(c.lh);
    const v2f32 recip2 = {lat.recip, lat.recip}, magic2 = {12582912.0f, 12582912.0f}, two_eb2 = {lat.two_eb, lat.two_eb};

    uint32_t ppA[TY], ppB[TY];
#pragma unroll
    for (int yy = 0; yy < TY; yy++) ppA[yy] = ppB[yy] = 0;

    auto fetch = [&](int zz, Q16Plane<TY> &R) {
        const float *src = c.in + (uint64_t)(z0 + (uint32_t)zz) * c.plane;
#pragma unroll
        for (int r = 0; r <= TY; r++) {
            const uint32_t gy = y0 + (uint32_t)r - 1u;
            R.rok[r] = gy < d1;
            if (R.rok[r]) {
                const float *row = src + (uint64_t)gy * d0;
#ifdef LAB_Q16_NTL
                {
                    typedef float f4v __attribute__((ext_vector_type(4)));
                    const f4v q = __builtin_nontemporal_load(reinterpret_cast<const f4v *>(row + lane_off));
                    R.rq[r] = make_float4(q.x, q.y, q.z, q.w);
                }
#else
                R.rq[r] = *reinterpret_cast<const float4 *>(row + lane_off);
#endif
                if (has_left) R.rl[r] = row[x0 - 1];
            }
        }
    };
    Q16Plane<TY> pa;
    auto work = [&](int zz, Q16Plane<TY> &R) {
        const uint32_t gz = z0 + (uint32_t)zz;
        uint32_t pd1A = 0, pd1B = 0;
        uint32_t bits_rows[(TY + 1) / 2];
#pragma unroll
        for (int k = 0; k < (TY + 1) / 2; k++) bits_rows[k] = 0;
        float qmax = 0.0f;
#pragma unroll
        for (int r = 0; r <= TY; r++) {
            uint32_t d1A = 0, d1B = 0;
            v2f32 s01 = {0.0f, 0.0f}, s23 = {0.0f, 0.0f}, t01 = magic2, t23 = magic2;
            if (R.rok[r]) {
                const v2f32 v01 = {R.rq[r].x, R.rq[r].y}, v23 = {R.rq[r].z, R.rq[r].w};
                s01 = v01 * recip2;
                s23 = v23 * recip2;
                t01 = s01 + magic2;
                t23 = s23 + magic2;
                uint32_t PA = pk_lo16(__float_as_uint(t01.x), __float_as_uint(t23.x));
                uint32_t PB = pk_lo16(__float_as_uint(t01.y), __float_as_uint(t23.y));
                if (EDGE) {
                    PA = xok ? PA : 0u;
                    PB = xok ? PB : 0u;
                }
                const uint32_t leftp = has_left ? __float_as_uint(R.rl[r] * lat.recip + 12582912.0f) << 16 : 0u;
                const uint32_t pv = (uint32_t)dpp_wave_shr1((int32_t)leftp, (int32_t)PB);
                const uint32_t XA = __builtin_amdgcn_alignbit(PB, pv, 16);
                d1A = pk_sub16(PA, XA);
                d1B = pk_sub16(PB, PA);
            }
            uint32_t sA = 0, sB = 0;
            if (r > 0) {
                const uint32_t d2A = pk_sub16(d1A, pd1A), d2B = pk_sub16(d1B, pd1B);
                sA = pk_sub16(d2A, ppA[r - 1]);
                sB = pk_sub16(d2B, ppB[r - 1]);
                ppA[r - 1] = d2A;
                ppB[r - 1] = d2B;
            }
            pd1A = d1A;
            pd1B = d1B;
            if (r == 0 || zz < 0) continue;
            if (!R.rok[r]) continue;
            const uint64_t grow = (uint64_t)gz * c.plane + (uint64_t)(y0 + r - 1) * d0;
            const uint32_t tqA = pk_add16(sA, 0x007F007Fu), tqB = pk_add16(sB, 0x007F007Fu);
            const uint32_t tA = pk_min16(tqA, 0x00FF00FFu), tB = pk_min16(tqB, 0x00FF00FFu);
            const uint32_t tm = pk_max16(tA, tB);
            const v2f32 r01 = t01 - magic2, r23 = t23 - magic2;
            const v2f32 v01 = {R.rq[r].x, R.rq[r].y}, v23 = {R.rq[r].z, R.rq[r].w};
            const v2f32 e01 = r01 * two_eb2 - v01, e23 = r23 * two_eb2 - v23;
            const bool b0 = !(fabsf(e01.x) <= lat.eb_lo), b1 = !(fabsf(e01.y) <= lat.eb_lo), b2 = !(fabsf(e23.x) <= lat.eb_lo), b3 = !(fabsf(e23.y) <= lat.eb_lo);
            qmax = fmaxf(fmaxf(qmax, fabsf(r01.x)), fabsf(r01.y));
            qmax = fmaxf(fmaxf(qmax, fabsf(r23.x)), fabsf(r23.y));
            bool rare = b0 | b1 | b2 | b3 | ((tm & 0xFFFFu) == 255u) | (tm >= 0x00FF0000u);
            if (EDGE) rare &= xok;
            const uint32_t a0 = mad16_lo(tA, c4), a1 = mad16_lo(tB, c4), a2 = mad16_hi(tA, c4), a3 = mad16_hi(tB, c4);
            if (!EDGE || xok) {
                if (!SAMP) {
                    atomicAdd(reinterpret_cast<uint32_t *>(lds + a0), 1u);
                    atomicAdd(reinterpret_cast<uint32_t *>(lds + a1), 1u);
                    atomicAdd(reinterpret_cast<uint32_t *>(lds + a2), 1u);
                    atomicAdd(reinterpret_cast<uint32_t *>(lds + a3), 1u);
                }
#if defined(LAB_ST) && LAB_ST == 1
                __hip_atomic_store(reinterpret_cast<uint32_t *>(c.codes8 + grow + x), tA | (tB << 8), __ATOMIC_RELAXED, __HIP_MEMORY_SCOPE_SYSTEM);
#elif defined(LAB_ST) && LAB_ST == 2
                *reinterpret_cast<uint32_t *>(c.codes8 + grow + x) = tA | (tB << 8);
#elif defined(LAB_ST) && LAB_ST == 3
                __hip_atomic_store(reinterpret_cast<uint32_t *>(c.codes8 + grow + x), tA | (tB << 8), __ATOMIC_RELAXED, __HIP_MEMORY_SCOPE_AGENT);
#else
                if (c.p->dbg & 8388608u) *reinterpret_cast<uint32_t *>(c.codes8 + grow + x) = tA | (tB << 8);
                else __builtin_nontemporal_store(tA | (tB << 8), reinterpret_cast<uint32_t *>(c.codes8 + grow + x));
#endif
            }
            if (SAMP ? c.have_len != 0u : c.s_len != nullptr) {
                uint32_t b4 = (uint32_t)lds[Q16_LEN_OFF + a0] + lds[Q16_LEN_OFF + a1] + lds[Q16_LEN_OFF + a2] + lds[Q16_LEN_OFF + a3];
                if (EDGE) b4 = xok ? b4 : 0u;
                bits_rows[(r - 1) >> 1] |= ((r - 1) & 1) ? b4 << 16 : b4;
            }
            if (__builtin_amdgcn_ballot_w64(rare)) {
                const bool bad[4] = {b0, b1, b2, b3};
                const float sv[4] = {s01.x, s01.y, s23.x, s23.y};
                const uint32_t t[4] = {tA & 0xFFFFu, tB & 0xFFFFu, tA >> 16, tB >> 16};
                const uint32_t delta[4] = {(uint32_t)(int32_t)(int16_t)(sA & 0xFFFFu), (uint32_t)(int32_t)(int16_t)(sB & 0xFFFFu),
                                           (uint32_t)(int32_t)(int16_t)(sA >> 16), (uint32_t)(int32_t)(int16_t)(sB >> 16)};
                uint32_t tmask = 0, badmask = 0;
                bool alien = false;
#pragma unroll
                for (int i = 0; i < 4; i++) {
                    tmask |= (uint32_t)(rare && t[i] == 255u) << i;
                    badmask |= (uint32_t)(rare && bad[i]) << i;
                    alien |= rare && bad[i] && !(fabsf(sv[i]) <= 4194304.0f);
                }
                if (alien) atomicOr(q16_flag, 1u);
                narrow_rare<float>(c, grow + x, delta, tmask, badmask);
            }
        }
        if (zz >= 0) {
            bool big = !(qmax <= Q16_LIM);
            if (EDGE) big &= xok;
            if (__builtin_amdgcn_ballot_w64(big)) {
                if (big) atomicOr(q16_flag, 1u);
            }
        }
        if ((SAMP ? c.have_len != 0u : c.s_len != nullptr) && zz >= 0) {
#pragma unroll
            for (int k = 0; k < (TY + 1) / 2; k++) {
                const uint32_t tot = wave_sum(bits_rows[k]);
                const uint32_t ra = y0 + 2u * k, rb = ra + 1u;
                if (lane == 0) {
                    const uint64_t g0 = (uint64_t)gz * c.plane + x0;
                    if (ra < d1) c.seg_bits[(g0 + (uint64_t)ra * d0) >> 8] = (uint16_t)(tot & 0xFFFFu);
                    if (2 * k + 1 < TY && rb < d1) c.seg_bits[(g0 + (uint64_t)rb * d0) >> 8] = (uint16_t)(tot >> 16);
                }
            }
        }
    };
    int zz = z0 > 0 ? -1 : 0;
    const int zend = d2 - z0 < (uint32_t)MARCH_TZ ? (int)(d2 - z0) : MARCH_TZ;
    auto put_len = [&](uint32_t b, uint32_t len) {
        uint32_t *lt = c.lh + NARROW_BINS * 4 + b * 4u;
        lt[0] = lt[1] = lt[2] = lt[3] = len;
    };
    auto catch_up = [&](int zhi) __attribute__((always_inline)) {
        asm volatile("s_waitcnt vmcnt(0)" ::: "memory");
        constexpr int PB = 4;
        for (int p0 = 0; p0 < zhi; p0 += PB) {
            uint32_t cw[PB][TY];
#pragma unroll
            for (int j = 0; j < PB; j++) {
                const uint64_t gp = (uint64_t)(z0 + (uint32_t)(p0 + j)) * c.plane;
#pragma unroll
                for (int r = 0; r < TY; r++) {
                    const uint32_t ry = y0 + (uint32_t)r;
                    cw[j][r] = 0x80808080u;
                    if (p0 + j < zhi && ry < d1 && xok)
                        cw[j][r] = __hip_atomic_load(reinterpret_cast<uint32_t *>(c.codes8 + gp + (uint64_t)ry * d0 + x), __ATOMIC_RELAXED, __HIP_MEMORY_SCOPE_WORKGROUP);
                }
            }
#pragma unroll
            for (int j = 0; j < PB; j++) {
                const uint64_t gp = (uint64_t)(z0 + (uint32_t)(p0 + j)) * c.plane;
                if (p0 + j < zhi)
#pragma unroll
                for (int k = 0; k < (TY + 1) / 2; k++) {
                    uint32_t packed = 0;
#pragma unroll
                    for (int h = 0; h < 2; h++) {
                        const uint32_t ry = y0 + 2u * k + h;
                        if (2 * k + h < TY && ry < d1 && xok) {
                            const uint32_t w = cw[j][(2 * k + h) < TY ? 2 * k + h : 0];
                            const uint32_t b4 = (uint32_t)lds[Q16_LEN_OFF + (w & 0xFFu) * 16u + c4] + lds[Q16_LEN_OFF + ((w >> 8) & 0xFFu) * 16u + c4] +
                                                lds[Q16_LEN_OFF + ((w >> 16) & 0xFFu) * 16u + c4] + lds[Q16_LEN_OFF + (w >> 24) * 16u + c4];
                            packed |= h ? b4 << 16 : b4;
                        }
                    }
                    const uint32_t tot = wave_sum(packed);
                    const uint32_t ra = y0 + 2u * k, rb = ra + 1u;
                    if (lane == 0) {
                        const uint64_t g0 = gp + x0;
                        if (ra < d1) c.seg_bits[(g0 + (uint64_t)ra * d0) >> 8] = (uint16_t)(tot & 0xFFFFu);
                        if (2 * k + 1 < TY && rb < d1) c.seg_bits[(g0 + (uint64_t)rb * d0) >> 8] = (uint16_t)(tot >> 16);
                    }
                }
            }
        }
    };
    if (SAMP) {
        for (; zz < zend; zz++) {
            fetch(zz, pa);
            work(zz, pa);
            if (!c.have_len && zz >= 0 && samp_poll(c, false, put_len)) catch_up(zz + 1);
        }
        if (!c.have_len) {
            samp_poll(c, true, put_len);
            catch_up(zend);
        }
        return;
    }
#if defined(LAB_Q16PF) && LAB_Q16PF == 1
    Q16Plane<TY> pb;
    fetch(zz, pa);
    for (;;) {
        if (zz + 1 < zend) fetch(zz + 1, pb);
        work(zz, pa);
        if (++zz >= zend) break;
        if (zz + 1 < zend) fetch(zz + 1, pa);
        work(zz, pb);
        if (++zz >= zend) break;
    }
#else
    for (; zz < zend; zz++) {
        fetch(zz, pa);
        work(zz, pa);
    }
#endif
}
template <int TY, bool SAMP>
__device__ __forceinline__ void march_narrow16(const float *__restrict__ in, uint16_t *__restrict__ codes, const szk_k1_params &p, uint32_t ntasks,
                                               uint32_t *lh, uint64_t (*s_oq_idx)[MarchLds<1, false>::OQ], uint32_t (*s_oq_val)[MarchLds<1, false>::OQ]) {
    const Lattice<float> lat(p.lat);
    NarrowCtx<float> c;
    c.in = in;
    c.codes8 = reinterpret_cast<uint8_t *>(codes);
    c.p = &p;
    c.d0 = (uint32_t)p.d[3];
    c.d1 = (uint32_t)p.d[2];
    c.d2 = (uint32_t)p.d[1];
    c.plane = (uint64_t)c.d1 * c.d0;
    c.vol = c.plane * c.d2;
    c.lh = lh;
    c.lane = lane_id();
    const uint32_t wv = (uint32_t)__builtin_amdgcn_readfirstlane((int)(threadIdx.x / WAVE));
    c.oq_idx = s_oq_idx[wv];
    c.oq_val = s_oq_val[wv];
    c.oq_n = 0;
    const bool acct = SAMP || (p.spec_lens != nullptr && c.d0 % MARCH_TX == 0);
    c.s_len = acct ? reinterpret_cast<const uint8_t *>(lh) + Q16_LEN_OFF : nullptr;
    c.seg_bits = p.seg_bits;
    c.s_enc = nullptr;
    c.stage = nullptr;
    c.slot = nullptr;
    c.slot_w = c.slot_base = c.st_cnt = 0;
    c.seg_base = p.seg_base;
    c.samp_words = p.samp.words;
// ... 1234 lines not shown
    if (w) keys[a] = mykey;
    __syncthreads();
    uint32_t r = 0;
    if (w)
        for (uint32_t o = 0; o < m; o++) r += keys[o] < mykey;
    __syncthreads();
    if (w) keys[r] = mykey;
    __syncthreads();
    if (t == 0) sp.info->ts[3] = wall_clock64();
    if (t < WAVE) cb_merge_wave32(keys, reinterpret_cast<uint32_t *>(ifreq), pleaf, pint, m);
    __syncthreads();
    if (t == 0) sp.info->ts[4] = wall_clock64();
    for (uint32_t q = t; q + 1 < m; q += CB_THREADS) {
        if (q == m - 2) pint[q] = (uint16_t)q;
        aux[q] = q == m - 2 ? 0 : 1;
    }
    __syncthreads();
    for (uint32_t span = 1; span < m && span < 2 * L; span <<= 1) {
        for (uint32_t q = t; q + 1 < m; q += CB_THREADS) {
            const uint16_t j = pint[q];
            const uint32_t sum = (uint32_t)aux[q] + aux[j];
            aux2[q] = (uint16_t)(sum > 0xFFFFu ? 0xFFFFu : sum);
            pint2[q] = pint[j];
        }
        __syncthreads();
        for (uint32_t q = t; q + 1 < m; q += CB_THREADS) {
            aux[q] = aux2[q];
            pint[q] = pint2[q];
        }
        __syncthreads();
    }
    if (t == 0) sp.info->ts[5] = wall_clock64();
    for (uint32_t q = t; q < m; q += CB_THREADS) {
        uint32_t l = (uint32_t)aux[pleaf[q]] + 1;
        if (l > L) {
            l = L;
            s_over = 1;
        }
        pleaf[q] = (uint16_t)l;
        atomicAdd(&s_cnt[l], 1u);
    }
    __syncthreads();
    if (s_over) cb_kraft_repair(pleaf, m, s_cnt, L, CB_THREADS, kraft_ws);
    s_l[t] = 0;
    __syncthreads();
    for (uint32_t q = t; q < m; q += CB_THREADS) s_l[(uint32_t)(keys[q] & 0xFFFFu)] = (uint8_t)pleaf[q];
    __syncthreads();
    if (t == 0) sp.info->ts[8] = wall_clock64();
    uint32_t ubits = 0;
    while ((1u << ubits) < n_un) ubits++;
    const uint32_t len = (n_un == 0 || cnt != 0) ? s_l[t] : (uint32_t)s_l[rep] + ubits;
    __syncthreads();
    s_l[t] = (uint8_t)len;
    uint32_t rank = 0;
    for (uint32_t l = 1; l <= SZH_MAX_LEN; l++) {
        const unsigned long long lm = __ballot(len == l);
        if (ln == 0) s_lc[wv][l] = (uint32_t)__popcll(lm);
        if (len == l) rank = (uint32_t)__popcll(lm & lower);
    }
    __syncthreads();
    if (t == 0) {
        uint32_t code = 0, maxl = 0, prev = 0;
        for (uint32_t l = 1; l <= SZH_MAX_LEN; l++) {
            const uint32_t c = s_lc[0][l] + s_lc[1][l] + s_lc[2][l] + s_lc[3][l];
            code = (code + prev) << (l > 1 ? 1 : 0);
            s_first[l] = code;
            prev = c;
            if (c) maxl = l;
        }
        sp.info->n_symbols = 256;
        sp.info->max_len = maxl;
        sp.info->sym_min = lo;
        sp.info->sym_count = 256;
        sp.info->win_lo = lo;
        sp.info->reserved = 0;
        sp.info->esc_sym = esc;
    }
    __syncthreads();
    for (uint32_t k = 0; k < wv; k++) rank += s_lc[k][len];
    const uint32_t e = ((s_first[len] + rank) << 5) | len;
    sp.enc[lo + t] = e;
    sp.lens[lo + t] = (uint8_t)len;
    if (t == 255) sp.enc[0] = e;
    if (t < 64) {
        const uint32_t w4 = (uint32_t)s_l[4 * t] | ((uint32_t)s_l[4 * t + 1] << 8) | ((uint32_t)s_l[4 * t + 2] << 16) | ((uint32_t)s_l[4 * t + 3] << 24);
        __hip_atomic_store(&sp.words[SZK_SAMP_LENS + t], w4, __ATOMIC_RELAXED, __HIP_MEMORY_SCOPE_AGENT);
    }
    asm volatile("s_waitcnt vmcnt(0)" ::: "memory");
    __syncthreads();
    if (t == 0) {
        __hip_atomic_store(&sp.words[SZK_SAMP_READY], 1u, __ATOMIC_RELAXED, __HIP_MEMORY_SCOPE_AGENT);
        sp.info->ts[10] = wall_clock64();
    }
}

template <typename T>
__global__ __launch_bounds__(256) void k_sample(const T *__restrict__ in, szk_k1_params p) {
    __shared__ __align__(16) uint32_t s_pool[(SAMP_POOL_BYTES + 3) / 4 > 1024 ? (SAMP_POOL_BYTES + 3) / 4 : 1024];
    if (!szk_is_narrow(p.mode)) return;
    if (samp_take<T>(in, p.lat, (uint32_t)p.d[3], (uint32_t)p.d[2], (uint32_t)p.d[1], p.samp.words, blockIdx.x, s_pool)) samp_book(p.samp, p.radius, reinterpret_cast<uint8_t *>(s_pool));
}

__global__ __launch_bounds__(1024) void k_cb_compact(const uint64_t *__restrict__ hist, uint64_t *__restrict__ keys, uint16_t *__restrict__ syms,
                                                     uint64_t *__restrict__ part) {
    __shared__ uint32_t s_w[16], s_before, s_oct[48];
    __shared__ unsigned long long s_sum;
    const uint32_t t = threadIdx.x, lane = lane_id(), wv = t / WAVE, w = blockIdx.x;
    if (t == 0) {
        s_before = 0;
        s_sum = 0;
    }
    if (t < 48) s_oct[t] = 0;
    __syncthreads();
    uint32_t before = 0;
    for (uint32_t b = 0; b < w; b++) before += hist[b * 1024u + t] != 0 ? 1u : 0u;
    before = wave_sum(before);
    if (lane == 0 && before) atomicAdd(&s_before, before);
    const uint32_t bin = w * 1024u + t;
    const uint64_t f = hist[bin];
    const unsigned long long bal = __ballot(f != 0);
    if (lane == 0) s_w[wv] = (uint32_t)__popcll(bal);
    const uint64_t fs = wave_sum(f);
    if (lane == 0 && fs) atomicAdd(&s_sum, (unsigned long long)fs);
    if (f) atomicAdd(&s_oct[(63 - __clzll((long long)f)) < 47 ? 63 - __clzll((long long)f) : 47], 1u);
    __syncthreads();
    if (t < 48) part[gridDim.x + 1 + w * 48u + t] = s_oct[t];
    uint32_t pos = s_before;
    for (uint32_t k = 0; k < wv; k++) pos += s_w[k];
    if (f) {
        const uint32_t at = pos + (uint32_t)__popcll(bal & ((1ull << lane) - 1ull));
        keys[at] = (f << 16) | bin;
        syms[at] = (uint16_t)bin;
    }
    if (t == 0) {
        part[w] = s_sum;
        if (w == gridDim.x - 1) {
            uint32_t m = s_before;
            for (uint32_t k = 0; k < 16; k++) m += s_w[k];
            part[gridDim.x] = m;
        }
    }
}
__global__ __launch_bounds__(1024) void k_cb_assign(const uint16_t *__restrict__ len_of, const uint16_t *__restrict__ syms, const szk_cb_info *__restrict__ info,
                                                    uint32_t *__restrict__ enc) {
    constexpr uint32_t NT = 1024;
    __shared__ uint16_t cnt_tbl[(SZH_MAX_LEN + 1) * NT];
// ... 362 lines not shown
                                 uint64_t *total_words, const uint16_t *__restrict__ seg_bits, uint64_t n_segs, const uint32_t *seg_made) {
    __shared__ uint64_t s_w[16];
    __shared__ uint64_t s_carry;
    const uint64_t n_groups = (n_chunks + PACK_GROUP - 1) / PACK_GROUP;
    if (threadIdx.x == 0) s_carry = 0;
    __syncthreads();
    for (uint64_t g0 = 0; g0 < n_groups; g0 += 1024 * SCAN_GPT) {
        const uint64_t gt = g0 + (uint64_t)threadIdx.x * SCAN_GPT;
        uint64_t sum[SCAN_GPT];
#pragma unroll
        for (int j = 0; j < SCAN_GPT; j++) {
            const uint64_t g = gt + j;
            sum[j] = 0;
            if (SEG) {
                sum[j] = g < n_groups ? reinterpret_cast<const uint32_t *>(seg_bits)[g] : 0u;
            } else if (g < n_groups) {
                const uint64_t c0 = g * PACK_GROUP;
                if (c0 + PACK_GROUP <= n_chunks) {
                    const uint4 *v = reinterpret_cast<const uint4 *>(chunk_words + c0);
                    uint4 q[4] = {v[0], v[1], v[2], v[3]};
#pragma unroll
                    for (int k = 0; k < 4; k++)
                        sum[j] += (q[k].x & 0xFFFF) + (q[k].x >> 16) + (q[k].y & 0xFFFF) + (q[k].y >> 16) + (q[k].z & 0xFFFF) +
                                  (q[k].z >> 16) + (q[k].w & 0xFFFF) + (q[k].w >> 16);
                } else {
                    for (uint64_t c = c0; c < n_chunks; c++) sum[j] += chunk_words[c];
                }
            }
        }
        uint64_t mine = 0;
#pragma unroll
        for (int j = 0; j < SCAN_GPT; j++) mine += sum[j];
        const uint64_t incl = wave_incl_scan(mine);
        if (lane_id() == WAVE - 1) s_w[threadIdx.x / WAVE] = incl;
        __syncthreads();
        uint64_t run = s_carry + incl - mine, tot = 0;
        for (int w = 0; w < 16; w++) {
            if (w < (int)(threadIdx.x / WAVE)) run += s_w[w];
            tot += s_w[w];
        }
#pragma unroll
        for (int j = 0; j < SCAN_GPT; j++) {
            if (gt + j < n_groups) group_off[gt + j] = run;
            run += sum[j];
        }
        __syncthreads();
        if (threadIdx.x == 0) s_carry += tot;
        __syncthreads();
    }
    if (threadIdx.x == 0) *total_words = s_carry;
}
__global__ __launch_bounds__(256) void k_seg_chunks(const uint16_t *__restrict__ seg_bits, uint64_t n_segs, const uint32_t *seg_made,
                                                    uint16_t *__restrict__ chunk_words, uint64_t n_chunks, uint32_t *__restrict__ group_sums,
                                                    uint16_t *__restrict__ sub_bits) {
    const bool seg_ok = *seg_made != 0;
    const uint64_t n_vec = (n_segs + 7) / 8;
    const uint64_t n_vec16 = (n_vec + 15) / 16 * 16;
    for (uint64_t vi = (uint64_t)blockIdx.x * 256 + threadIdx.x; vi < n_vec16; vi += (uint64_t)gridDim.x * 256) {
        const uint4 q = vi < n_vec ? reinterpret_cast<const uint4 *>(seg_bits)[vi] : make_uint4(0, 0, 0, 0);
        const uint64_t sg0 = vi * 8;
        uint32_t hw[8] = {q.x & 0xFFFF, q.x >> 16, q.y & 0xFFFF, q.y >> 16, q.z & 0xFFFF, q.z >> 16, q.w & 0xFFFF, q.w >> 16};
#pragma unroll
        for (int k = 0; k < 8; k++) hw[k] = (seg_ok && sg0 + k < n_segs) ? hw[k] : 0u;
        const uint32_t cw0 = (hw[0] + hw[1] + hw[2] + hw[3] + 31u) >> 5, cw1 = (hw[4] + hw[5] + hw[6] + hw[7] + 31u) >> 5;
        const uint64_t c = vi * 2;
        if (c + 1 < n_chunks) reinterpret_cast<uint32_t *>(chunk_words)[vi] = cw0 | (cw1 << 16);
        else if (c < n_chunks) chunk_words[c] = (uint16_t)cw0;
        if (sub_bits) {
            constexpr uint32_t SPU = 4 / SZH_SUBS;
#pragma unroll
            for (uint32_t h = 0; h < 2; h++) {
                uint32_t run = 0;
#pragma unroll
                for (uint32_t u = 1; u < SZH_SUBS; u++) {
#pragma unroll
                    for (uint32_t q = 0; q < SPU; q++) run += hw[4 * h + (u - 1) * SPU + q];
                    if (c + h < n_chunks) sub_bits[(c + h) * (SZH_SUBS - 1) + u - 1] = (uint16_t)run;
                }
            }
        }
        uint32_t gs = (c < n_chunks ? cw0 : 0u) + (c + 1 < n_chunks ? cw1 : 0u);
        gs += dpp_mov0<0x111, 0xf>(gs);
        gs += dpp_mov0<0x112, 0xf>(gs);
        gs += dpp_mov0<0x114, 0xf>(gs);
        gs += dpp_mov0<0x118, 0xf>(gs);
        if ((lane_id() & 15) == 15) group_sums[vi >> 4] = gs;
    }
}
struct szk_fold_params {
    const uint32_t *partial;
    uint32_t nrows;
    int win_lo;
    uint64_t *hist;
    uint32_t *range;
};
__global__ __launch_bounds__(1024) void k_scan_groups(uint16_t *__restrict__ chunk_words, uint64_t n_chunks,
                                                      uint64_t *__restrict__ group_off, uint64_t *total_words,
                                                      szk_layout_params lp, int do_layout, const uint16_t *__restrict__ seg_bits, uint64_t n_segs,
                                                      const uint32_t *seg_made, szk_fold_params fp) {
    if (blockIdx.x > 0) {
        const int bin = threadIdx.x;
        uint64_t sum = 0;
        for (uint32_t r = blockIdx.x - 1; r < fp.nrows; r += gridDim.x - 1) sum += fp.partial[(uint64_t)r * HIST_WIN + bin];
        const int sym = fp.win_lo + bin;
        if (sum && sym >= 0 && sym < (int)SZH_HIST_BINS) hist_add_ranged(fp.hist, fp.range, (uint32_t)sym, (unsigned long long)sum);
        return;
    }
// ... 53 lines not shown
            const uint32_t l1 = e1 & 31u;
            if (G == 4) pc[h] = ((e0 >> 5) << l1) | (e1 >> 5);
            else pc[h] = ((uint64_t)(e0 >> 5) << l1) | (e1 >> 5);
            pl[h] = (e0 & 31u) + l1;
        }
        if (G == 4) {
            g[k] = (pc[0] << pl[G / 2 - 1]) | pc[G / 2 - 1];
            gl[k] = pl[0] + pl[G / 2 - 1];
        } else {
            g[k] = pc[0];
            gl[k] = pl[0];
        }
        bits += gl[k];
    }
    const uint32_t incl = wave_incl_scan(bits);
    const uint32_t total_bits = (uint32_t)__builtin_amdgcn_readlane((int)incl, WAVE - 1);
    uint32_t pos = incl - bits;
    if (BYTE && G == 4) {
        const bool fits = gl[0] + gl[1] <= 64u && gl[2] + gl[3] <= 64u;
        if (!__builtin_amdgcn_ballot_w64(!fits)) {
#pragma unroll
            for (int k = 0; k < NG; k += 2) {
                const uint32_t len = gl[k] + gl[k + 1];
                const uint64_t joined = (gl[k + 1] < 64u ? g[k] << gl[k + 1] : 0ull) | g[k + 1];
                const uint64_t v = len ? joined << (64 - len) : 0ull;
                const uint32_t word = pos >> 5, sh = pos & 31;
                const uint64_t t = v >> sh;
#if defined(LAB_PACK) && (LAB_PACK & 2)
                if (t == 0x123456789ull) stage[word] = 1;
#else
                atomicOr(&stage[word], (uint32_t)(t >> 32));
                atomicOr(&stage[word + 1], (uint32_t)t);
                atomicOr(&stage[word + 2], (uint32_t)(((uint64_t)(uint32_t)v << 32) >> sh));
#endif
                pos += len;
            }
            return (total_bits + 31) >> 5;
        }
    }
#pragma unroll
    for (int k = 0; k < NG; k++) {
        const uint64_t v = gl[k] ? g[k] << (64 - gl[k]) : 0ull;
        const uint32_t word = pos >> 5, sh = pos & 31;
        const uint64_t t = v >> sh;
        const uint32_t w2 = (uint32_t)(((uint64_t)(uint32_t)v << 32) >> sh);
        atomicOr(&stage[word], (uint32_t)(t >> 32));
        atomicOr(&stage[word + 1], (uint32_t)t);
        if (G == 4 || gl[k] + sh > 64) atomicOr(&stage[word + 2], w2);
        pos += gl[k];
    }
    return (total_bits + 31) >> 5;
}

__device__ void assemble_body(const szk_asm_params &p, uint64_t tid, uint64_t nth) {
    __shared__ szh_header s_h0, s_h;
    __shared__ szh_offsets s_o, s_oo;
    if (threadIdx.x == 0) {
        s_h0 = p.state->hdr;
        s_o = p.state->off;
    }
    __syncthreads();
    const szh_header &h0 = s_h0;
    const szh_offsets &o = s_o;
    if (tid == 0) {
        szh_header &h = s_h;
        szh_offsets &oo = s_oo;
        h = s_h0;
        h.bitstream_words = *p.total_words;
        szh_compute_offsets(h, oo);
        h.payload_bytes = oo.end;
        *reinterpret_cast<szh_header *>(p.payload) = h;
        p.state->hdr = h;
        p.state->off = oo;
        p.state->cap_exceeded = oo.end > p.cap;
        for (int i = 0; i < 6; i++) p.state->probe[i] = reinterpret_cast<const uint32_t *>(p.n_vout + 4)[i];
        if (p.assumed_narrow && !szk_is_narrow(p.mode)) atomicOr(&p.state->miss_kind, 32u);
        if (p.q16_flag && *p.q16_flag) atomicOr(&p.state->miss_kind, 128u);
        if (p.samp_words && p.samp_words[SZK_SAMP_READY]) {
            p.state->mispredict = 0;
            p.state->book_miss = 0;
            p.state->n_symbols = 256;
        } else if (!p.lists_by_roles) {
            p.state->mispredict = (uint32_t)p.n_vout[7];
            p.state->book_miss = 0;
            p.state->n_symbols = reinterpret_cast<const uint32_t *>(p.n_vout + 8)[2];
        }
        const uint64_t tsz0 = h.dtype == 0 ? 4 : 8;
        for (uint64_t a = oo.lens + h.sym_count; a < oo.chunkwords; a++) p.payload[a] = 0;
        for (uint64_t a = oo.chunkwords + 2 * h.n_chunks; a < oo.subbits; a++) p.payload[a] = 0;
        for (uint64_t a = oo.subbits + 2 * (SZH_SUBS - 1) * h.n_chunks; a < oo.vout_idx; a++) p.payload[a] = 0;
        for (uint64_t a = oo.vout_val + tsz0 * h.n_vout; a < oo.dout_idx; a++) p.payload[a] = 0;
        for (uint64_t a = oo.dout_val + (uint64_t)h.qbytes * h.n_dout; a < oo.side; a++) p.payload[a] = 0;
        for (uint64_t a = oo.side + (h.predictor == 2 ? h.side_bytes : 0); a < oo.bitstream; a++) p.payload[a] = 0;
    }
    for (uint64_t i = tid; i < h0.sym_count; i += nth) p.payload[o.lens + i] = p.lens[h0.sym_min + i];
    uint16_t *cw = reinterpret_cast<uint16_t *>(p.payload + o.chunkwords);
    for (uint64_t i = tid; i < h0.n_chunks; i += nth) cw[i] = p.chunk_words[i];
    uint16_t *sb = reinterpret_cast<uint16_t *>(p.payload + o.subbits);
    for (uint64_t i = tid; i < h0.n_chunks * (SZH_SUBS - 1); i += nth) sb[i] = p.sub_bits[i];
}
__device__ void assemble_lists(const szk_asm_params &p, uint64_t tid, uint64_t nth) {
    const uint64_t n_vout = p.state->hdr.n_vout, n_dout = p.state->hdr.n_dout;
    const uint32_t dtype = p.state->hdr.dtype, qbytes = p.state->hdr.qbytes, predictor = p.state->hdr.predictor;
    const uint64_t side_bytes = p.state->hdr.side_bytes;
    const uint64_t o_vi = p.state->off.vout_idx, o_vv = p.state->off.vout_val, o_di = p.state->off.dout_idx, o_dv = p.state->off.dout_val,
                   o_side = p.state->off.side;
    uint64_t *vi = reinterpret_cast<uint64_t *>(p.payload + o_vi);
    uint64_t *di = reinterpret_cast<uint64_t *>(p.payload + o_di);
    for (uint64_t i = tid; i < n_vout; i += nth) vi[i] = p.vout_idx[i];
    for (uint64_t i = tid; i < n_dout; i += nth) di[i] = p.dout_idx[i];
    if (dtype == 0) {
        uint32_t *d = reinterpret_cast<uint32_t *>(p.payload + o_vv);
        for (uint64_t i = tid; i < n_vout; i += nth) d[i] = reinterpret_cast<const uint32_t *>(p.vout_val)[i];
    } else {
        uint64_t *d = reinterpret_cast<uint64_t *>(p.payload + o_vv);
        for (uint64_t i = tid; i < n_vout; i += nth) d[i] = reinterpret_cast<const uint64_t *>(p.vout_val)[i];
    }
    if (qbytes == 4) {
        uint32_t *d = reinterpret_cast<uint32_t *>(p.payload + o_dv);
        for (uint64_t i = tid; i < n_dout; i += nth) d[i] = reinterpret_cast<const uint32_t *>(p.dout_val)[i];
    } else if (qbytes == 8) {
// ... 248 lines not shown
#pragma unroll
            for (int i = 0; i < 16; i++) c[i] = (uint16_t)((wds[i >> 2] >> (8 * (i & 3))) & 0xFFu);
            nwords = pack_chunk<4, true>(c, 0, 0, false, s_enc8, g_enc, sym_min, all_lds, stage, s_plen8);
        } else {
            unpack_codes(cur, narrow, sym_add, c);
            nwords = wide ? pack_chunk<2, false, WIN>(c, 0, 0, false, s_enc, g_enc, sym_min, all_lds, stage)
                          : pack_chunk<4, false, WIN>(c, 0, 0, false, s_enc, g_enc, sym_min, all_lds, stage);
        }
        const uint32_t before = wave_sum(bp_cur);
        __builtin_amdgcn_fence(__ATOMIC_RELEASE, "workgroup");
        __builtin_amdgcn_wave_barrier();
        uint32_t *out = out_base + go_cur + before;
        for (uint32_t i = 2 * lane; i < nwords + 2; i += 2 * WAVE) {
            const uint2 wv = *reinterpret_cast<const uint2 *>(&stage[i]);
            *reinterpret_cast<uint2 *>(&stage[i]) = make_uint2(0u, 0u);
#if defined(LAB_PACK) && (LAB_PACK & 4)
            if (wv.x == 0x12345678u && wv.y == 0x9abcdef0u) out[i] = 1;
#else
#ifdef LAB_PACK_NT
            if (i < nwords) __builtin_nontemporal_store(__builtin_bswap32(wv.x), &out[i]);
            if (i + 1 < nwords) __builtin_nontemporal_store(__builtin_bswap32(wv.y), &out[i + 1]);
#else
            if (i < nwords) out[i] = __builtin_bswap32(wv.x);
            if (i + 1 < nwords) out[i + 1] = __builtin_bswap32(wv.y);
#endif
#endif
        }
        __builtin_amdgcn_wave_barrier();
        cur = nxt;
        bp_cur = bp_nxt;
        go_cur = go_nxt;
    }
    if (n_full < n_chunks && wave_gid == 0) {
        const uint64_t base = n_full * SZH_CHUNK_SYMS + lane_off;
        uint16_t c[ENC_PER_LANE];
        load_codes16(codes, base, n, narrow, sym_add, c);
        uint32_t bp;
        uint64_t go;
        side(n_full, bp, go);
        const uint32_t nwords = wide ? pack_chunk<2, false, WIN>(c, base, n, true, s_enc, g_enc, sym_min, all_lds, stage)
                                     : pack_chunk<4, false, WIN>(c, base, n, true, s_enc, g_enc, sym_min, all_lds, stage);
        const uint32_t before = wave_sum(bp);
        __builtin_amdgcn_fence(__ATOMIC_RELEASE, "workgroup");
        __builtin_amdgcn_wave_barrier();
        uint32_t *out = out_base + go + before;
        for (uint32_t i = lane; i < nwords; i += WAVE) out[i] = __builtin_bswap32(stage[i]);
    }
    if (nblk > pack_blocks && !ap.lists_by_roles) assemble_lists(ap, (uint64_t)bid * 256 + threadIdx.x, (uint64_t)nblk * 256);
}

#define PB_THREADS 1024u
#define PB_WAVES (PB_THREADS / WAVE)
#define PB_ASM_BLOCKS 32u
__device__ __forceinline__ void packb_emit(uint64_t *stage, uint64_t val, uint32_t len, uint32_t pos) {
    const uint64_t v = val << ((64u - len) & 63u);
    const uint32_t q = pos >> 6, sh = pos & 63u;
    atomicOr(reinterpret_cast<unsigned long long *>(&stage[q]), (unsigned long long)(v >> sh));
    atomicOr(reinterpret_cast<unsigned long long *>(&stage[q + 1]), (unsigned long long)((v << 1) << (63u - sh)));
}
__device__ __forceinline__ uint32_t packb_chunk(const uint4 &cw, const uint32_t *__restrict__ s_pair, const uint32_t *__restrict__ s_enc8,
                                                const uint8_t *__restrict__ s_len8, uint64_t *stage) {
    const uint32_t w[4] = {cw.x, cw.y, cw.z, cw.w};
    {
        constexpr uint32_t K = 0x40404040u;
        const uint32_t inw = (w[0] + K) & (w[1] + K) & (w[2] + K) & (w[3] + K) & 0x80808080u;
        uint32_t e[8];
#pragma unroll
        for (int k = 0; k < 4; k++) {
            const uint32_t m = w[k] & 0x7F7F7F7Fu, x = m ^ (m >> 8), m1 = m >> 16, x1 = x >> 16;
            const uint32_t a0 = ((x & 0x7Fu) << 2) | ((m & 0x7F00u) << 1), a1 = ((x1 & 0x7Fu) << 2) | ((m1 & 0x7F00u) << 1);
            e[2 * k] = *reinterpret_cast<const uint32_t *>(reinterpret_cast<const uint8_t *>(s_pair) + a0);
            e[2 * k + 1] = *reinterpret_cast<const uint32_t *>(reinterpret_cast<const uint8_t *>(s_pair) + a1);
        }
        const uint32_t emin = min(min(min(e[0], e[1]), min(e[2], e[3])), min(min(e[4], e[5]), min(e[6], e[7])));
        uint64_t O[2];
        uint32_t OL[2];
#pragma unroll
        for (int i = 0; i < 2; i++) {
            const uint32_t l0 = e[4 * i] & 31u, l1 = e[4 * i + 1] & 31u, l2 = e[4 * i + 2] & 31u, l3 = e[4 * i + 3] & 31u;
            const uint64_t qa = ((uint64_t)(e[4 * i] >> 5) << l1) | (e[4 * i + 1] >> 5);
            const uint64_t qb = ((uint64_t)(e[4 * i + 2] >> 5) << l3) | (e[4 * i + 3] >> 5);
            const uint32_t lb = l2 + l3;
            OL[i] = l0 + l1 + lb;
            O[i] = (qa << (lb & 63u)) | qb;
        }
        const bool fast = inw == 0x80808080u && emin != 0u && OL[0] <= 64u && OL[1] <= 64u;
        if (!__builtin_amdgcn_ballot_w64(!fast)) {
            const uint32_t bits = OL[0] + OL[1];
            const uint32_t incl = wave_incl_scan(bits);
            const uint32_t total_bits = (uint32_t)__builtin_amdgcn_readlane((int)incl, WAVE - 1);
            const uint32_t pos = incl - bits;
            packb_emit(stage, O[0], OL[0], pos);
            packb_emit(stage, O[1], OL[1], pos + OL[0]);
            return (total_bits + 31u) >> 5;
        }
    }
    uint64_t P[8];
    uint32_t PL[8];
#pragma unroll
    for (int k = 0; k < 8; k++) {
        const uint32_t pr = (w[k >> 1] >> (16 * (k & 1))) & 0xFFFFu;
        const uint32_t b0 = pr & 0xFFu, b1 = pr >> 8;
        const uint32_t l1 = s_len8[b1];
        P[k] = ((uint64_t)s_enc8[b0] << l1) | s_enc8[b1];
        PL[k] = (uint32_t)s_len8[b0] + l1;
    }
    uint64_t Q[4];
    uint32_t QL[4];
    bool fit_q = true;
#pragma unroll
    for (int j = 0; j < 4; j++) {
        QL[j] = PL[2 * j] + PL[2 * j + 1];
        Q[j] = (P[2 * j] << (PL[2 * j + 1] & 63u)) | P[2 * j + 1];
        fit_q &= QL[j] <= 64u;
    }
    const bool fit_o = QL[0] + QL[1] <= 64u && QL[2] + QL[3] <= 64u;
    const uint32_t bits = QL[0] + QL[1] + QL[2] + QL[3];
    const uint32_t incl = wave_incl_scan(bits);
    const uint32_t total_bits = (uint32_t)__builtin_amdgcn_readlane((int)incl, WAVE - 1);
    uint32_t pos = incl - bits;
    if (!__builtin_amdgcn_ballot_w64(!fit_o)) {
#pragma unroll
        for (int i = 0; i < 2; i++) {
            const uint32_t len = QL[2 * i] + QL[2 * i + 1];
            if (len) packb_emit(stage, (Q[2 * i] << (QL[2 * i + 1] & 63u)) | Q[2 * i + 1], len, pos);
            pos += len;
        }
    } else if (!__builtin_amdgcn_ballot_w64(!fit_q)) {
#pragma unroll
        for (int j = 0; j < 4; j++) {
            if (QL[j]) packb_emit(stage, Q[j], QL[j], pos);
            pos += QL[j];
        }
    } else {
#pragma unroll
        for (int k = 0; k < 8; k++) {
            if (PL[k]) packb_emit(stage, P[k], PL[k], pos);
            pos += PL[k];
        }
    }
    return (total_bits + 31u) >> 5;
}
__global__ __launch_bounds__(PB_THREADS) void k_pack_b(const uint16_t *__restrict__ codes, uint64_t n, const uint32_t *__restrict__ g_enc,
                                                        const uint16_t *__restrict__ chunk_words, const uint64_t *__restrict__ group_off, szk_mode mode,
                                                        uint32_t sym_add, const szk_state *__restrict__ state, uint8_t *__restrict__ payload,
                                                        szk_asm_params ap, uint32_t pack_blocks, uint32_t split, szk_role_params rp, uint32_t only_sampled) {
    constexpr int STAGE_WORDS = SZH_CHUNK_SYMS * SZH_MAX_LEN / 32 + 4;
    __shared__ __align__(16) uint32_t s_pair[128 * 128];
    __shared__ uint32_t s_enc8[256];
    __shared__ uint8_t s_plen8[256];
    __shared__ __align__(8) uint64_t s_stage[PB_WAVES][STAGE_WORDS / 2];
    if ((only_sampled & 1u) && !(ap.samp_words && ap.samp_words[SZK_SAMP_READY] && szk_is_narrow(mode))) return;
    const uint32_t roles = rp.on ? ROLE_BLOCKS : 0u;
    if (blockIdx.x < roles) {
        if (threadIdx.x >= 256u) return;
        if (blockIdx.x != 0) role_sort(rp, ap, blockIdx.x == 2, reinterpret_cast<uint8_t *>(s_pair));
        return;
    }
    const uint32_t asm_blocks = gridDim.x - roles - pack_blocks;
    if (blockIdx.x >= roles + pack_blocks) {
        const uint32_t ab = blockIdx.x - roles - pack_blocks;
        assemble_body(ap, (uint64_t)ab * PB_THREADS + threadIdx.x, (uint64_t)asm_blocks * PB_THREADS);
        if (!ap.lists_by_roles) assemble_lists(ap, (uint64_t)ab * PB_THREADS + threadIdx.x, (uint64_t)asm_blocks * PB_THREADS);
        return;
    }
    const uint32_t bid = blockIdx.x - roles;
    if (!szk_is_narrow(mode)) return;
    const uint64_t n_full = n / SZH_CHUNK_SYMS, n_chunks = (n + SZH_CHUNK_SYMS - 1) / SZH_CHUNK_SYMS;
    (void)split;
    const uint32_t wv = threadIdx.x / WAVE;
    const uint64_t wave_gid = (uint64_t)bid * PB_WAVES + wv, nwaves = (uint64_t)pack_blocks * PB_WAVES;
    const int lane = lane_id();
    const uint8_t *c8 = reinterpret_cast<const uint8_t *>(codes) + (uint64_t)lane * ENC_PER_LANE;
    uint64_t *stage = s_stage[wv];
    uint32_t *out_base = reinterpret_cast<uint32_t *>(payload + state->off.bitstream);
    constexpr uint32_t PB_BATCH = 4;
    const uint64_t n_units = (n_full + PB_BATCH - 1) / PB_BATCH;
#ifdef SZ3HIP_LAB
    const bool lab_nost = (only_sampled & 8u) != 0, lab_nold = (only_sampled & 16u) != 0;
#else
    constexpr bool lab_nost = false, lab_nold = false;
#endif
    auto fetch = [&](uint64_t ch) { return ch < n_full ? *reinterpret_cast<const uint4 *>(c8 + (lab_nold ? ch % (4 * nwaves) : ch) * SZH_CHUNK_SYMS) : make_uint4(0u, 0u, 0u, 0u); };
    auto front_of = [&](uint64_t unit) -> uint32_t {
        const uint64_t c_lo = unit * PB_BATCH, grp = c_lo / PACK_GROUP;
        const uint32_t first = (uint32_t)(c_lo % PACK_GROUP);
        return ((uint32_t)lane < first && grp * PACK_GROUP + lane < n_chunks) ? chunk_words[grp * PACK_GROUP + lane] : 0u;
    };
    uint64_t unit = wave_gid;
    uint4 cur[PB_BATCH], nxt[PB_BATCH];
    uint32_t fr_cur = 0, fr_nxt = 0;
    uint64_t go_cur = 0, go_nxt = 0;
#pragma unroll
    for (uint32_t j = 0; j < PB_BATCH; j++) cur[j] = make_uint4(0u, 0u, 0u, 0u);
    if (unit < n_units) {
#pragma unroll
        for (uint32_t j = 0; j < PB_BATCH; j++) cur[j] = fetch(unit * PB_BATCH + j);
        fr_cur = front_of(unit);
        go_cur = group_off[unit * PB_BATCH / PACK_GROUP];
    }
    if (threadIdx.x < 256u) {
        const uint32_t e = g_enc[threadIdx.x != 255u ? threadIdx.x + sym_add : 0u];
        s_enc8[threadIdx.x] = e >> 5;
        s_plen8[threadIdx.x] = (uint8_t)(e & 31u);
    }
    for (int i = lane; i < STAGE_WORDS / 2; i += WAVE) stage[i] = 0;
    __syncthreads();
    for (uint32_t i = threadIdx.x; i < 128u * 128u; i += PB_THREADS) {
        const uint32_t i1 = i >> 7, i0 = (i & 127u) ^ i1;
        const uint32_t t0 = i0 < 64u ? i0 + 128u : i0, t1 = i1 < 64u ? i1 + 128u : i1;
        const uint32_t l0 = s_plen8[t0], l1 = s_plen8[t1];
        const uint32_t len = l0 + l1;
        s_pair[i] = (l0 && l1 && len <= 27u) ? ((((s_enc8[t0] << l1) | s_enc8[t1]) << 5) | len) : 0u;
    }
    __syncthreads();
    for (; unit < n_units; unit += nwaves) {
        const uint64_t nu = unit + nwaves;
        if (nu < n_units) {
#pragma unroll
            for (uint32_t j = 0; j < PB_BATCH; j++) nxt[j] = fetch(nu * PB_BATCH + j);
            fr_nxt = front_of(nu);
            go_nxt = group_off[nu * PB_BATCH / PACK_GROUP];
        }
        uint32_t *out = out_base + go_cur + wave_sum(fr_cur);
        const uint64_t c_lo = unit * PB_BATCH;
#pragma unroll
        for (uint32_t j = 0; j < PB_BATCH; j++) {
            if (c_lo + j < n_full) {
                const uint32_t nwords = packb_chunk(cur[j], s_pair, s_enc8, s_plen8, stage);
                __builtin_amdgcn_fence(__ATOMIC_RELEASE, "workgroup");
                __builtin_amdgcn_wave_barrier();
                for (uint32_t i = 2 * lane; i < nwords + 2; i += 2 * WAVE) {
                    const uint64_t v = stage[i >> 1];
                    stage[i >> 1] = 0;
                    if (lab_nost && v != 0x123456789abcdefull) continue;
                    if (i < nwords) out[i] = __builtin_bswap32((uint32_t)(v >> 32));
                    if (i + 1 < nwords) out[i + 1] = __builtin_bswap32((uint32_t)v);
                }
                __builtin_amdgcn_wave_barrier();
                out += nwords;
            }
        }
#pragma unroll
        for (uint32_t j = 0; j < PB_BATCH; j++) cur[j] = nxt[j];
        fr_cur = fr_nxt;
        go_cur = go_nxt;
    }
    if (n_full < n_chunks && wave_gid == 0) {
        const uint64_t base = n_full * SZH_CHUNK_SYMS + (uint64_t)lane * ENC_PER_LANE;
        const uint8_t *cb = reinterpret_cast<const uint8_t *>(codes);
        uint32_t bits = 0;
        uint64_t P[8];
        uint32_t PL[8];
#pragma unroll
        for (int k = 0; k < 8; k++) {
            const uint64_t i0 = base + 2 * k, i1 = i0 + 1;
            const uint32_t b0 = i0 < n ? cb[i0] : 0u, b1 = i1 < n ? cb[i1] : 0u;
            const uint32_t l0 = i0 < n ? s_plen8[b0] : 0u, l1 = i1 < n ? s_plen8[b1] : 0u;
            P[k] = ((uint64_t)(i0 < n ? s_enc8[b0] : 0u) << l1) | (i1 < n ? s_enc8[b1] : 0u);
            PL[k] = l0 + l1;
            bits += PL[k];
        }
        const uint32_t incl = wave_incl_scan(bits);
        const uint32_t total_bits = (uint32_t)__builtin_amdgcn_readlane((int)incl, WAVE - 1);
        uint32_t pos = incl - bits;
#pragma unroll
        for (int k = 0; k < 8; k++) {
            if (PL[k]) packb_emit(stage, P[k], PL[k], pos);
            pos += PL[k];
        }
        const uint32_t nwords = (total_bits + 31u) >> 5;
        const uint64_t grp = n_full / PACK_GROUP;
        const uint32_t cin = (uint32_t)(n_full % PACK_GROUP);
        uint32_t bp = (uint32_t)lane < cin ? chunk_words[grp * PACK_GROUP + lane] : 0u;
        const uint32_t before = wave_sum(bp);
        __builtin_amdgcn_fence(__ATOMIC_RELEASE, "workgroup");
        __builtin_amdgcn_wave_barrier();
        uint32_t *out = out_base + group_off[grp] + before;
        for (uint32_t i = lane; i < nwords; i += WAVE) out[i] = __builtin_bswap32((uint32_t)(stage[i >> 1] >> ((i & 1u) ? 0 : 32)));
    }
}

#ifdef SZ3HIP_LAB
struct szk_merge_params {
    const uint32_t *slots;
    const uint16_t *seg_bits;
    const uint32_t *seg_base;
    const uint32_t *fuse_flag;
};
#define MERGE_BLOCK 16
__global__ __launch_bounds__(256) void k_merge(szk_merge_params mp, uint64_t n, const uint16_t *__restrict__ chunk_words,
                                               const uint64_t *__restrict__ group_off, szk_mode mode, const szk_state *__restrict__ state,
                                               uint8_t *__restrict__ payload, szk_asm_params ap, uint32_t pack_blocks, szk_role_params rp) {
    __shared__ __align__(16) uint32_t s_pool[ENC_WIN];
    const uint32_t roles = rp.on ? ROLE_BLOCKS : 0u;
    if (blockIdx.x < roles) {
        if (blockIdx.x == 0) {
#if defined(LAB_MERGE) && (LAB_MERGE & 1)
            if (threadIdx.x == 0) { ap.state->mispredict = 0; ap.state->n_symbols = rp.cb.range[2]; }
#else
            if (!rp.no_book) role_book(rp, ap.state, reinterpret_cast<uint8_t *>(s_pool));
#endif
            if (threadIdx.x == 0 && *mp.fuse_flag) atomicOr(&ap.state->miss_kind, 64u);
        } else role_sort(rp, ap, blockIdx.x == 2, reinterpret_cast<uint8_t *>(s_pool));
        return;
    }
    const uint32_t bid = blockIdx.x - roles;
    const uint32_t nblk = gridDim.x - roles;
    if (bid >= pack_blocks) {
        assemble_body(ap, (uint64_t)(bid - pack_blocks) * 256 + threadIdx.x, (uint64_t)(nblk - pack_blocks) * 256);
        if (!ap.lists_by_roles) assemble_lists(ap, (uint64_t)bid * 256 + threadIdx.x, (uint64_t)nblk * 256);
        return;
    }
    if (ap.assumed_narrow && !szk_is_narrow(mode)) return;
    const uint64_t n_chunks = (n + SZH_CHUNK_SYMS - 1) / SZH_CHUNK_SYMS, n_segs = n >> 8;
    const uint64_t n_blocks = (n_chunks + MERGE_BLOCK - 1) / MERGE_BLOCK;
    const uint64_t wave_gid = (uint64_t)bid * 4 + threadIdx.x / WAVE, nwaves = (uint64_t)pack_blocks * 4;
    const int lane = lane_id();
    uint32_t *out_base = reinterpret_cast<uint32_t *>(payload + state->off.bitstream);
#if defined(LAB_MERGE) && (LAB_MERGE & 2)
    if (n_blocks) return;
#endif
    for (uint64_t blk = wave_gid; blk < n_blocks; blk += nwaves) {
        const uint64_t chunk0 = blk * MERGE_BLOCK;
        const uint64_t seg = chunk0 * 4 + (uint64_t)lane;
        const bool seg_ok = seg < n_segs;
        const uint32_t sb = seg_ok ? mp.seg_bits[seg] : 0u;
        const uint32_t sa = seg_ok ? mp.seg_base[seg] : 0u;
        const uint64_t grp = chunk0 / PACK_GROUP;
        const uint64_t gc = grp * PACK_GROUP + (uint64_t)(lane & 31);
        const uint32_t cw = (lane < 32 && gc < n_chunks) ? chunk_words[gc] : 0u;
// ... 1445 lines not shown
int szk_launch_codebook(const uint64_t *d_hist, const szk_cb_params *p, hipStream_t s) {
    const uint32_t nb = p->n_books ? p->n_books : 1;
    szk_cb_params q = *p;
    q.n_books = nb;
    q.dbg = ((szk_dbg_flags & 1024) ? 1u : 0u) | ((szk_dbg_flags & 262144) ? 2u : 0u);
    if (nb > 1) {
        hipError_t e = hipMemsetAsync(q.range, 0, 16 * nb, s);
        if (e != hipSuccess) return (int)e;
    }
    if (!p->range_ready) hipLaunchKernelGGL(k_hist_range, dim3(SZH_HIST_BINS / 256, nb), dim3(256), 0, s, d_hist, q.range);
    q.keys_ready = nb == 1 && p->part_hint != 0 && !(szk_dbg_flags & 1) ? 1 : 0;
    if (q.keys_ready) hipLaunchKernelGGL(k_cb_compact, dim3(CBC_BLOCKS), dim3(1024), 0, s, d_hist, q.keys, q.syms, q.ifreq);
    if (p->part_hint != 1) hipLaunchKernelGGL(k_codebook<0>, dim3(nb == 1 ? 3 : nb), dim3(CB_LAUNCH), 0, s, d_hist, q);
    q.assign_later = q.keys_ready;
    if (p->part_hint != 0) hipLaunchKernelGGL(k_codebook<1>, dim3(nb == 1 ? 3 : nb), dim3(CB_LAUNCH), 0, s, d_hist, q);
    if (p->part_hint != 0 && q.assign_later) hipLaunchKernelGGL(k_cb_assign, dim3(16), dim3(1024), 0, s, (const uint16_t *)q.depth, (const uint16_t *)q.syms, (const szk_cb_info *)q.info, q.enc);
    SZK_CHECK_LAUNCH();
    return 0;
}
__global__ __launch_bounds__(1024) void k_book_verdict(const szk_cb_info *__restrict__ fresh, const uint8_t *__restrict__ fresh_lens,
                                                       const szk_cb_info *__restrict__ used, const uint8_t *__restrict__ used_lens,
                                                       const uint32_t *__restrict__ mispredict, const uint32_t *__restrict__ range, szk_state *state,
                                                       const uint64_t *__restrict__ hist, int exact) {
    __shared__ uint32_t s_diff;
    __shared__ unsigned long long s_acc[3];
    if (threadIdx.x == 0) s_diff = 0;
    if (threadIdx.x < 3) s_acc[threadIdx.x] = 0;
    __syncthreads();
    const bool built = *mispredict == 0;
    if (built && book_rejected(hist, fresh, fresh_lens, used, used_lens, exact != 0, threadIdx.x, 1024u, s_acc) && threadIdx.x == 0) s_diff = 1;
    __syncthreads();
    if (threadIdx.x == 0) {
        atomicOr(&state->miss_kind, (s_diff ? 1u : 0u) | (!built ? 2u : 0u));
        state->mispredict = built ? 0u : 1u;
        state->n_symbols = range[2];
    }
}
int szk_launch_book_verdict(const szk_cb_info *fresh, const uint8_t *fresh_lens, const szk_cb_info *used, const uint8_t *used_lens,
                            const uint32_t *mispredict, const uint32_t *range, szk_state *state, const uint64_t *hist, int exact, hipStream_t s) {
    hipLaunchKernelGGL(k_book_verdict, dim3(1), dim3(1024), 0, s, fresh, fresh_lens, used, used_lens, mispredict, range, state, hist, exact);
    SZK_CHECK_LAUNCH();
    return 0;
}
int szk_launch_hist_range(const uint64_t *d_hist, uint32_t *range, hipStream_t s) {
    hipLaunchKernelGGL(k_hist_range, dim3(SZH_HIST_BINS / 256, 1), dim3(256), 0, s, d_hist, range);
    SZK_CHECK_LAUNCH();
    return 0;
}
int szk_launch_hist_fold(const uint32_t *partial, uint32_t nrows, int radius, uint64_t *hist, uint32_t *range, hipStream_t s) {
    hipLaunchKernelGGL(k_hist_reduce, dim3(HIST_WIN / 256, 64), dim3(256), 0, s, partial, nrows, radius - HIST_WIN / 2, hist, range);
    SZK_CHECK_LAUNCH();
    return 0;
}
int szk_launch_encode(const uint16_t *codes, uint64_t n, const uint32_t *d_enc, const szk_cb_info *info, int radius,
                      szk_mode mode, uint16_t *chunk_words, uint64_t *group_off, uint64_t *total_words,
                      const szk_state *state, uint8_t *payload, const szk_layout_params *layout, const szk_asm_params *asmp, hipStream_t s,
                      const uint16_t *seg_bits, const uint32_t *seg_made, const szk_encode_roles *er, const szk_merge_args *mg) {
    const uint64_t n_chunks = (n + SZH_CHUNK_SYMS - 1) / SZH_CHUNK_SYMS;
    const uint64_t nb = (n_chunks + 3) / 4;
    if (nb > 0x7FFFFFFFull) return -1;
    const uint32_t sym_add = (uint32_t)radius - 127u;
    const uint32_t pgrid = (uint32_t)(nb < 2048 ? nb : 2048);
    uint16_t *sub_bits = asmp ? asmp->sub_bits : nullptr;
    if (!seg_bits) hipLaunchKernelGGL(k_chunk_bits2, dim3(pgrid), dim3(256), 0, s, codes, n, d_enc, info, mode, sym_add, chunk_words, sub_bits);
    szk_fold_params fp{};
    if (er && er->fold_rows) {
        fp.partial = er->fold_partial;
        fp.nrows = er->fold_rows;
        fp.win_lo = radius - HIST_WIN / 2;
        fp.hist = er->fold_hist;
        fp.range = er->fold_range;
    }
    const uint16_t *scan_in = nullptr;
    if (seg_bits) {
        const uint64_t n_segs = (n + 255) / 256;
        uint32_t *gsums = reinterpret_cast<uint32_t *>(group_off + (n_chunks + PACK_GROUP - 1) / PACK_GROUP + 1);
        hipLaunchKernelGGL(k_seg_chunks, dim3((uint32_t)std::min<uint64_t>(((n_segs + 7) / 8 + 255) / 256, 1024)), dim3(256), 0, s, seg_bits, n_segs, seg_made,
                           chunk_words, n_chunks, gsums, sub_bits);
        scan_in = reinterpret_cast<const uint16_t *>(gsums);
    }
    hipLaunchKernelGGL(k_scan_groups, dim3(fp.nrows ? 65 : 1), dim3(1024), 0, s, chunk_words, n_chunks, group_off, total_words, *layout, 1, scan_in,
                       (uint64_t)0, seg_made, fp);
    szk_role_params rp{};
    szk_asm_params apv = asmp ? *asmp : szk_asm_params{};
    if (er && er->roles && asmp) {
        rp.on = 1;
        rp.no_book = er->no_book ? 1u : 0u;
        rp.hist = er->hist;
        rp.cb = *er->cb;
        rp.used = info;
        rp.used_lens = er->used_lens;
        rp.flags = er->flags;
        rp.need_seg = seg_bits != nullptr;
        rp.exact = er->exact;
        apv.lists_by_roles = 1;
    }
    const uint32_t rb = rp.on ? ROLE_BLOCKS : 0u;
    const uint32_t extra = rb + (asmp ? 32u : 0u);
    constexpr uint32_t ASM_BLOCKS = 32;
#ifdef SZ3HIP_LAB
    if (mg) {
        szk_merge_params mp;
        mp.slots = mg->slots;
        mp.seg_bits = seg_bits;
        mp.seg_base = mg->seg_base;
        mp.fuse_flag = mg->fuse_flag;
        const uint32_t pb = pgrid < 2048 - extra ? pgrid : 2048 - extra;
        hipLaunchKernelGGL(k_merge, dim3(rb + pb + (asmp ? ASM_BLOCKS : 0)), dim3(256), 0, s, mp, n, chunk_words, group_off, mode, state, payload, apv, pb, rp);
    } else
#else
    if (mg) return -2;
#endif
    if (asmp && !(rp.on && !rp.no_book) && n_chunks >= 4096 && ((asmp->assumed_narrow && !(szk_dbg_flags & 32768)) || asmp->samp_words)) {
        static int n_cu = 0;
        if (!n_cu) {
            int dev = 0;
            hipDeviceProp_t prop;
            if (hipGetDevice(&dev) == hipSuccess && hipGetDeviceProperties(&prop, dev) == hipSuccess) n_cu = prop.multiProcessorCount;
            if (n_cu <= 0) n_cu = 256;
        }
        const uint32_t pb = (uint32_t)n_cu > rb + 1 ? (uint32_t)n_cu - rb : 1u;
        const uint32_t split = 1;
        uint32_t beside = asmp->samp_words && !asmp->assumed_narrow ? 1u : 0u;
#ifdef SZ3HIP_LAB
        beside |= (szk_dbg_flags & 16) ? 8u : 0u;
        beside |= (szk_dbg_flags & 512) ? 16u : 0u;
#endif
        hipLaunchKernelGGL(k_pack_b, dim3(rb + PB_ASM_BLOCKS + pb), dim3(PB_THREADS), 0, s, codes, n, d_enc, chunk_words, group_off, mode, sym_add, state,
                           payload, apv, pb, split, rp, beside);
        if (beside & 1u) {
            const uint32_t pb2 = pgrid < 1280 - extra ? pgrid : 1280 - extra;
            hipLaunchKernelGGL((k_pack<ENC_WIN>), dim3(rb + pb2 + (asmp ? ASM_BLOCKS : 0)), dim3(256), 0, s, codes, n, d_enc, info, chunk_words, group_off, mode,
                               sym_add, state, payload, apv, pb2, rp);
        }
    } else if (mode.pack_wide) {
        const uint32_t pb = pgrid < 768 - extra ? pgrid : 768 - extra;
        hipLaunchKernelGGL((k_pack<2 * ENC_WIN>), dim3(rb + pb + (asmp ? ASM_BLOCKS : 0)), dim3(256), 0, s, codes, n, d_enc, info, chunk_words, group_off, mode,
                           sym_add, state, payload, apv, pb, rp);
    } else {
        const uint32_t pb = pgrid < 1280 - extra ? pgrid : 1280 - extra;
        hipLaunchKernelGGL((k_pack<ENC_WIN>), dim3(rb + pb + (asmp ? ASM_BLOCKS : 0)), dim3(256), 0, s, codes, n, d_enc, info, chunk_words, group_off, mode,
                           sym_add, state, payload, apv, pb, rp);
    }
    SZK_CHECK_LAUNCH();
    return 0;
}
__global__ __launch_bounds__(256) void k_publish(const szk_state *__restrict__ state, uint32_t *host_state, uint32_t *host_seq, uint32_t seq,
                                                 uint4 *zero, uint32_t zero_vec16, const uint64_t *blk_others, uint4 *zero_blk0, uint4 *zero_blk1) {
    if (blockIdx.x == 0) {
        const uint32_t *src = reinterpret_cast<const uint32_t *>(state);
        constexpr uint32_t OW = offsetof(szk_state, blk_others) / 4;
        for (uint32_t i = threadIdx.x; i < sizeof(szk_state) / 4; i += 256) {
            uint32_t v = src[i];
            if (blk_others && (i == OW || i == OW + 1)) v = reinterpret_cast<const uint32_t *>(blk_others)[i - OW];
            __hip_atomic_store(&host_state[i], v, __ATOMIC_RELAXED, __HIP_MEMORY_SCOPE_SYSTEM);
        }
        __threadfence_system();
        __syncthreads();
        if (threadIdx.x == 0) __hip_atomic_store(host_seq, seq, __ATOMIC_RELEASE, __HIP_MEMORY_SCOPE_SYSTEM);
        if (zero && zero_blk0 && state->miss_kind == 0 && state->mispredict == 0) {
            if (threadIdx.x < 4) zero_blk0[threadIdx.x] = make_uint4(0u, 0u, 0u, 0u);
            else if (threadIdx.x < 9) zero_blk1[threadIdx.x - 4] = make_uint4(0u, 0u, 0u, 0u);
        }
    }
    if (zero && state->miss_kind == 0 && state->mispredict == 0)
        for (uint32_t i = blockIdx.x * 256 + threadIdx.x; i < zero_vec16; i += gridDim.x * 256) zero[i] = make_uint4(0u, 0u, 0u, 0u);
}
int szk_launch_publish(const szk_state *d_state, void *h_state, uint32_t *h_seq, uint32_t seq, void *d_zero, uint64_t zero_bytes, hipStream_t s,
                       const uint64_t *d_blk_others, void *d_zero_blk0, void *d_zero_blk1) {
    static_assert(sizeof(szk_state) % 4 == 0, "the state block is copied word by word");
    hipLaunchKernelGGL(k_publish, dim3(d_zero ? 128 : 1), dim3(256), 0, s, d_state, (uint32_t *)h_state, h_seq, seq, (uint4 *)d_zero, (uint32_t)(zero_bytes / 16),
                       d_blk_others, (uint4 *)d_zero_blk0, (uint4 *)d_zero_blk1);
    SZK_CHECK_LAUNCH();
    return 0;
}
int szk_launch_assemble(const szk_asm_params *p, hipStream_t s) {
    hipLaunchKernelGGL(k_assemble, dim3(512), dim3(256), 0, s, *p);
    SZK_CHECK_LAUNCH();
    return 0;
}

int szk_launch_dec_tables(const uint8_t *d_lens, uint32_t sym_min, uint32_t sym_count, szk_dec_tables *t, uint32_t radius, uint32_t esc_sym, uint32_t *zero_word,
// ... 220 lines not shown
```

Before: 2279 GB/s.

## Fold group scan into packer, keep early code window, publish sampled lengths earlier

Removes the separate k_scan_groups launch when sampled narrow encoding applies. The packer blocks instead scan the per-group sums in LDS, and the assembler computes the total itself; layout_pre moves into k_seg_chunks. The Q16 stage keeps the first 8 planes of codes in registers so catch-up does not reread global memory, and the ready flag is loaded before the plane's work. The sampled-book kernel also publishes lengths and the ready flag before building encodings, and the packer writes pairs of output words with 64-bit stores. This adds register pressure and a bounded group count, plus a new sample-hold debug knob.

```diff
diff --git a/include/sz3hip.h b/include/sz3hip.h
--- a/include/sz3hip.h
+++ b/include/sz3hip.h
@@ -127,6 +127,11 @@
 void sz3hip_get_spec_stats(const sz3hip_ctx *ctx, uint32_t *hits, uint32_t *misses);
 int sz3hip_last_call_fused(const sz3hip_ctx *ctx);
 int sz3hip_last_call_q16(const sz3hip_ctx *ctx);
+#define SZ3HIP_FORM_SAMPLED_IN_LAUNCH 1u
+#define SZ3HIP_FORM_CODE_WINDOW 2u
+#define SZ3HIP_FORM_SCAN_IN_PACKER 4u
+int sz3hip_last_call_forms(const sz3hip_ctx *ctx);
+void sz3hip_ctx_set_sample_hold(sz3hip_ctx *ctx, unsigned microseconds);
 void sz3hip_ctx_set_fused(sz3hip_ctx *ctx, int on);
 int sz3hip_lab_build(void);
 int sz3hip_debug_copy_codes(sz3hip_ctx *ctx, uint16_t *host_codes, uint64_t n);
diff --git a/sz3_amd/__init__.py b/sz3_amd/__init__.py
--- a/sz3_amd/__init__.py
+++ b/sz3_amd/__init__.py
@@ -4,6 +4,7 @@
 import numpy as np
 
 _HERE = os.path.dirname(os.path.abspath(__file__))
+FORM_SAMPLED_IN_LAUNCH, FORM_CODE_WINDOW, FORM_SCAN_IN_PACKER = 1, 2, 4
 LIB_PATH = os.environ.get("SZ3HIP_LIB") or os.path.join(_HERE, "libsz3hip.so")
 
 EB_ABS, EB_REL, EB_PSNR, EB_L2NORM, EB_ABS_AND_REL, EB_ABS_OR_REL = range(6)
@@ -166,6 +167,11 @@
     L.sz3hip_last_call_fused.restype = C.c_int
     L.sz3hip_last_call_q16.argtypes = [C.c_void_p]
     L.sz3hip_last_call_q16.restype = C.c_int
+    if hasattr(L, "sz3hip_last_call_forms"):
+        L.sz3hip_last_call_forms.argtypes = [C.c_void_p]
+        L.sz3hip_last_call_forms.restype = C.c_int
+        L.sz3hip_ctx_set_sample_hold.argtypes = [C.c_void_p, C.c_uint]
+        L.sz3hip_ctx_set_sample_hold.restype = None
     L.sz3hip_ctx_set_fused.argtypes = [C.c_void_p, C.c_int]
     L.sz3hip_ctx_set_fused.restype = None
     L.sz3hip_get_spec_stats.argtypes = [C.c_void_p, C.POINTER(C.c_uint32), C.POINTER(C.c_uint32)]
@@ -493,6 +499,13 @@
     def q16(self):
         return bool(lib().sz3hip_last_call_q16(self._h))
 
+    @property
+    def forms(self):
+        return int(lib().sz3hip_last_call_forms(self._h))
+
+    def set_sample_hold(self, microseconds):
+        lib().sz3hip_ctx_set_sample_hold(self._h, int(microseconds))
+
     def spec_stats(self):
         h, m = C.c_uint32(), C.c_uint32()
         lib().sz3hip_get_spec_stats(self._h, C.byref(h), C.byref(m))
diff --git a/sz3_amd/csrc/sz3hip_api.cpp b/sz3_amd/csrc/sz3hip_api.cpp
--- a/sz3_amd/csrc/sz3hip_api.cpp
+++ b/sz3_amd/csrc/sz3hip_api.cpp
@@ -580,6 +580,7 @@
         p.samp.enc = ctx->bk[fresh].enc;
         p.samp.lens = ctx->bk[fresh].lens;
         p.samp.info = ctx->bk[fresh].info;
+        p.samp.hold_ticks = ctx->samp_hold_us * 100u;
         p.seg_bits = ctx->d_seg_bits;
         p.seg_made = reinterpret_cast<uint32_t *>(ctx->d_counters + 10) + 1;
     }
@@ -1689,6 +1690,7 @@
                                (fused || wide || how == S2_SAMPLED) ? &er : nullptr, merge ? &mg : nullptr);
     prof_end(ctx, ST_ENCODE, s);
     if (rc) return fail(SZ3HIP_EHIP, "encode kernel launch failed (%d)", rc);
+    ctx->s2_pack_scan = szk_encode_scans_in_packer(n, &ap, (fused || (samp_words && ctx->s1_samp_in)) && ctx->seg_expected, how == S2_SAMPLED ? &er : nullptr);
     if (wide) {
         HIPCHK(hipStreamWaitEvent(s, ctx->ev_book, 0));
         if (szk_launch_book_verdict(ctx->bk[fresh].info, ctx->bk[fresh].lens, ctx->bk[used].info, ctx->bk[used].lens,
@@ -1802,6 +1804,8 @@
         if (int rw = wait_published(ctx)) return rw;
         if (ctx->h_state->mispredict) return fail(SZ3HIP_EHIP, "code book was not built (both forms declined)");
     }
+    ctx->last_forms = (ctx->s1_samp_in ? SZ3HIP_FORM_SAMPLED_IN_LAUNCH : 0u) | (ctx->s1_samp_in && ctx->s1_q16 ? SZ3HIP_FORM_CODE_WINDOW : 0u) |
+                      (ctx->s2_pack_scan ? SZ3HIP_FORM_SCAN_IN_PACKER : 0u);
     ctx->stage1_done = ctx->stage2_done = false;
     if (ctx->pub_zero && ctx->h_state->miss_kind == 0 && ctx->h_state->mispredict == 0) {
         ctx->pre_cleared = true;
@@ -2021,6 +2025,8 @@
 }
 extern "C" int sz3hip_last_call_fused(const sz3hip_ctx *ctx) { return ctx->last_fused ? 1 : 0; }
 extern "C" int sz3hip_last_call_q16(const sz3hip_ctx *ctx) { return ctx->last_q16 ? 1 : 0; }
+extern "C" int sz3hip_last_call_forms(const sz3hip_ctx *ctx) { return (int)ctx->last_forms; }
+extern "C" void sz3hip_ctx_set_sample_hold(sz3hip_ctx *ctx, unsigned microseconds) { ctx->samp_hold_us = microseconds > 1000u ? 1000u : microseconds; }
 extern "C" int sz3hip_lab_build(void) {
 #ifdef SZ3HIP_LAB
     return 1;
diff --git a/sz3_amd/csrc/sz3hip_internal.h b/sz3_amd/csrc/sz3hip_internal.h
--- a/sz3_amd/csrc/sz3hip_internal.h
+++ b/sz3_amd/csrc/sz3hip_internal.h
@@ -74,6 +74,9 @@
     int q16_block;
     bool s1_q16;
     bool last_q16;
+    uint32_t last_forms;
+    bool s2_pack_scan;
+    uint32_t samp_hold_us;
     bool range_ready;
     bool hist_exposed;
     int half_skip;
diff --git a/sz3_amd/csrc/sz3hip_kernels.h b/sz3_amd/csrc/sz3hip_kernels.h
--- a/sz3_amd/csrc/sz3hip_kernels.h
+++ b/sz3_amd/csrc/sz3hip_kernels.h
@@ -46,6 +46,7 @@
     uint32_t *enc;
     uint8_t *lens;
     szk_cb_info *info;
+    uint32_t hold_ticks;
 };
 struct szk_k1_params {
     uint64_t d[4];
@@ -321,6 +322,7 @@
 int szk_launch_minmax(int dtype, const void *d_in, uint64_t n, double *d_partial , double *d_out , hipStream_t s);
 int szk_launch_k1(int dtype, int ndim, const void *d_in, uint16_t *codes, szk_k1_params *p, hipStream_t s);
 int szk_launch_codebook(const uint64_t *d_hist, const szk_cb_params *p, hipStream_t s);
+bool szk_encode_scans_in_packer(uint64_t n, const szk_asm_params *asmp, bool seg, const szk_encode_roles *er);
 int szk_launch_encode(const uint16_t *codes, uint64_t n, const uint32_t *d_enc, const szk_cb_info *info, int radius,
                       szk_mode mode, uint16_t *chunk_words, uint64_t *group_off , uint64_t *total_words,
                       const szk_state *state, uint8_t *payload, const szk_layout_params *layout,
diff --git a/sz3_amd/csrc/sz3hip_kernels.hip b/sz3_amd/csrc/sz3hip_kernels.hip
--- a/sz3_amd/csrc/sz3hip_kernels.hip
+++ b/sz3_amd/csrc/sz3hip_kernels.hip
@@ -926,8 +926,11 @@
 template <typename T> __device__ __forceinline__ bool samp_take(const T *__restrict__ in, const szk_lattice &latp, uint32_t d0, uint32_t d1, uint32_t d2, uint32_t *words, uint32_t role, uint32_t *s_h);
 __device__ __forceinline__ void samp_book(const szk_samp &sp, uint32_t radius, uint8_t *pool);
 #define SAMP_POOL_BYTES (SZK_CB_SMALL_SYMS * 28 + 256)
-template <typename T, typename PUT>
-__device__ __forceinline__ bool samp_poll(NarrowCtx<T> &c, bool spin, PUT put) {
+__device__ __forceinline__ uint32_t samp_ask(const uint32_t *samp_words) {
+    return __hip_atomic_load(const_cast<uint32_t *>(samp_words) + SZK_SAMP_READY, __ATOMIC_RELAXED, __HIP_MEMORY_SCOPE_AGENT);
+}
+template <typename T, typename PUT, bool EARLY = false>
+__device__ __forceinline__ bool samp_poll(NarrowCtx<T> &c, bool spin, PUT put, uint32_t early = 0u) {
     volatile uint32_t *s_have = c.s_have;
     const uint32_t wv = (uint32_t)__builtin_amdgcn_readfirstlane((int)(threadIdx.x / WAVE));
     if (wv != 0) {
@@ -943,7 +946,7 @@
         c.have_len = 1;
         return true;
     }
-    uint32_t r = __hip_atomic_load(const_cast<uint32_t *>(c.samp_words) + SZK_SAMP_READY, __ATOMIC_RELAXED, __HIP_MEMORY_SCOPE_AGENT);
+    uint32_t r = EARLY ? early : samp_ask(c.samp_words);
     r = (uint32_t)__builtin_amdgcn_readfirstlane((int)r);
     if (!r) {
         if (!spin) return false;
@@ -1475,6 +1478,7 @@
     return d;
 }
 #define Q16_LEN_OFF (NARROW_BINS * 16)
+#define Q16_WIN_PLANES 8
 template <int TY> struct Q16Plane {
     float4 rq[TY + 1];
     float rl[TY + 1];
@@ -1518,6 +1522,13 @@
         }
     };
     Q16Plane<TY> pa;
+    uint32_t win[Q16_WIN_PLANES][TY];
+    if (SAMP) {
+#pragma unroll
+        for (int j = 0; j < Q16_WIN_PLANES; j++)
+#pragma unroll
+            for (int r = 0; r < TY; r++) win[j][r] = 0x80808080u;
+    }
     auto work = [&](int zz, Q16Plane<TY> &R) {
         const uint32_t gz = z0 + (uint32_t)zz;
         uint32_t pd1A = 0, pd1B = 0;
@@ -1590,6 +1601,10 @@
                 else __builtin_nontemporal_store(tA | (tB << 8), reinterpret_cast<uint32_t *>(c.codes8 + grow + x));
 #endif
             }
+            if (SAMP && c.have_len == 0u && zz < Q16_WIN_PLANES) {
+#pragma unroll
+                for (int j = 0; j < Q16_WIN_PLANES; j++) win[j][r - 1] = zz == j ? (tA | (tB << 8)) : win[j][r - 1];
+            }
             if (SAMP ? c.have_len != 0u : c.s_len != nullptr) {
                 uint32_t b4 = (uint32_t)lds[Q16_LEN_OFF + a0] + lds[Q16_LEN_OFF + a1] + lds[Q16_LEN_OFF + a2] + lds[Q16_LEN_OFF + a3];
                 if (EDGE) b4 = xok ? b4 : 0u;
@@ -1639,10 +1654,38 @@
         uint32_t *lt = c.lh + NARROW_BINS * 4 + b * 4u;
         lt[0] = lt[1] = lt[2] = lt[3] = len;
     };
+    auto sum_plane = [&](int pz, const uint32_t (&cw)[TY]) __attribute__((always_inline)) {
+        const uint64_t gp = (uint64_t)(z0 + (uint32_t)pz) * c.plane;
+#pragma unroll
+        for (int k = 0; k < (TY + 1) / 2; k++) {
+            uint32_t packed = 0;
+#pragma unroll
+            for (int h = 0; h < 2; h++) {
+                const uint32_t ry = y0 + 2u * k + h;
+                if (2 * k + h < TY && ry < d1 && xok) {
+                    const uint32_t w = cw[(2 * k + h) < TY ? 2 * k + h : 0];
+                    const uint32_t b4 = (uint32_t)lds[Q16_LEN_OFF + (w & 0xFFu) * 16u + c4] + lds[Q16_LEN_OFF + ((w >> 8) & 0xFFu) * 16u + c4] +
+                                        lds[Q16_LEN_OFF + ((w >> 16) & 0xFFu) * 16u + c4] + lds[Q16_LEN_OFF + (w >> 24) * 16u + c4];
+                    packed |= h ? b4 << 16 : b4;
+                }
+            }
+            const uint32_t tot = wave_sum(packed);
+            const uint32_t ra = y0 + 2u * k, rb = ra + 1u;
+            if (lane == 0) {
+                const uint64_t g0 = gp + x0;
+                if (ra < d1) c.seg_bits[(g0 + (uint64_t)ra * d0) >> 8] = (uint16_t)(tot & 0xFFFFu);
+                if (2 * k + 1 < TY && rb < d1) c.seg_bits[(g0 + (uint64_t)rb * d0) >> 8] = (uint16_t)(tot >> 16);
+            }
+        }
+    };
     auto catch_up = [&](int zhi) __attribute__((always_inline)) {
+#pragma unroll
+        for (int j = 0; j < Q16_WIN_PLANES; j++)
+            if (j < zhi) sum_plane(j, win[j]);
+        if (zhi <= Q16_WIN_PLANES) return;
         asm volatile("s_waitcnt vmcnt(0)" ::: "memory");
         constexpr int PB = 4;
-        for (int p0 = 0; p0 < zhi; p0 += PB) {
+        for (int p0 = Q16_WIN_PLANES; p0 < zhi; p0 += PB) {
             uint32_t cw[PB][TY];
 #pragma unroll
             for (int j = 0; j < PB; j++) {
@@ -1656,38 +1699,19 @@
                 }
             }
 #pragma unroll
-            for (int j = 0; j < PB; j++) {
-                const uint64_t gp = (uint64_t)(z0 + (uint32_t)(p0 + j)) * c.plane;
-                if (p0 + j < zhi)
-#pragma unroll
-                for (int k = 0; k < (TY + 1) / 2; k++) {
-                    uint32_t packed = 0;
-#pragma unroll
-                    for (int h = 0; h < 2; h++) {
-                        const uint32_t ry = y0 + 2u * k + h;
-                        if (2 * k + h < TY && ry < d1 && xok) {
-                            const uint32_t w = cw[j][(2 * k + h) < TY ? 2 * k + h : 0];
-                            const uint32_t b4 = (uint32_t)lds[Q16_LEN_OFF + (w & 0xFFu) * 16u + c4] + lds[Q16_LEN_OFF + ((w >> 8) & 0xFFu) * 16u + c4] +
-                                                lds[Q16_LEN_OFF + ((w >> 16) & 0xFFu) * 16u + c4] + lds[Q16_LEN_OFF + (w >> 24) * 16u + c4];
-                            packed |= h ? b4 << 16 : b4;
-                        }
-                    }
-                    const uint32_t tot = wave_sum(packed);
-                    const uint32_t ra = y0 + 2u * k, rb = ra + 1u;
-                    if (lane == 0) {
-                        const uint64_t g0 = gp + x0;
-                        if (ra < d1) c.seg_bits[(g0 + (uint64_t)ra * d0) >> 8] = (uint16_t)(tot & 0xFFFFu);
-                        if (2 * k + 1 < TY && rb < d1) c.seg_bits[(g0 + (uint64_t)rb * d0) >> 8] = (uint16_t)(tot >> 16);
-                    }
-                }
-            }
+            for (int j = 0; j < PB; j++)
+                if (p0 + j < zhi) sum_plane(p0 + j, cw[j]);
         }
     };
     if (SAMP) {
+        const bool wave0 = __builtin_amdgcn_readfirstlane((int)(threadIdx.x / WAVE)) == 0;
         for (; zz < zend; zz++) {
+            const bool ask = !c.have_len && zz >= 0;
+            uint32_t ready = 0;
+            if (ask && wave0) ready = samp_ask(c.samp_words);
             fetch(zz, pa);
             work(zz, pa);
-            if (!c.have_len && zz >= 0 && samp_poll(c, false, put_len)) catch_up(zz + 1);
+            if (ask && samp_poll<float, decltype(put_len), true>(c, false, put_len, ready)) catch_up(zz + 1);
         }
         if (!c.have_len) {
             samp_poll(c, true, put_len);
@@ -3028,6 +3052,21 @@
     const uint32_t len = (n_un == 0 || cnt != 0) ? s_l[t] : (uint32_t)s_l[rep] + ubits;
     __syncthreads();
     s_l[t] = (uint8_t)len;
+    __syncthreads();
+    if (t < 64) {
+        const uint32_t w4 = (uint32_t)s_l[4 * t] | ((uint32_t)s_l[4 * t + 1] << 8) | ((uint32_t)s_l[4 * t + 2] << 16) | ((uint32_t)s_l[4 * t + 3] << 24);
+        __hip_atomic_store(&sp.words[SZK_SAMP_LENS + t], w4, __ATOMIC_RELAXED, __HIP_MEMORY_SCOPE_AGENT);
+    }
+    asm volatile("s_waitcnt vmcnt(0)" ::: "memory");
+    __syncthreads();
+    if (t == 0) {
+        if (sp.hold_ticks) {
+            const uint64_t t0 = wall_clock64();
+            while (wall_clock64() - t0 < (uint64_t)sp.hold_ticks) __builtin_amdgcn_s_sleep(32);
+        }
+        __hip_atomic_store(&sp.words[SZK_SAMP_READY], 1u, __ATOMIC_RELAXED, __HIP_MEMORY_SCOPE_AGENT);
+        sp.info->ts[10] = wall_clock64();
+    }
     uint32_t rank = 0;
     for (uint32_t l = 1; l <= SZH_MAX_LEN; l++) {
         const unsigned long long lm = __ballot(len == l);
@@ -3058,16 +3097,6 @@
     sp.enc[lo + t] = e;
     sp.lens[lo + t] = (uint8_t)len;
     if (t == 255) sp.enc[0] = e;
-    if (t < 64) {
-        const uint32_t w4 = (uint32_t)s_l[4 * t] | ((uint32_t)s_l[4 * t + 1] << 8) | ((uint32_t)s_l[4 * t + 2] << 16) | ((uint32_t)s_l[4 * t + 3] << 24);
-        __hip_atomic_store(&sp.words[SZK_SAMP_LENS + t], w4, __ATOMIC_RELAXED, __HIP_MEMORY_SCOPE_AGENT);
-    }
-    asm volatile("s_waitcnt vmcnt(0)" ::: "memory");
-    __syncthreads();
-    if (t == 0) {
-        __hip_atomic_store(&sp.words[SZK_SAMP_READY], 1u, __ATOMIC_RELAXED, __HIP_MEMORY_SCOPE_AGENT);
-        sp.info->ts[10] = wall_clock64();
-    }
 }
 
 template <typename T>
@@ -3536,7 +3565,8 @@
 }
 __global__ __launch_bounds__(256) void k_seg_chunks(const uint16_t *__restrict__ seg_bits, uint64_t n_segs, const uint32_t *seg_made,
                                                     uint16_t *__restrict__ chunk_words, uint64_t n_chunks, uint32_t *__restrict__ group_sums,
-                                                    uint16_t *__restrict__ sub_bits) {
+                                                    uint16_t *__restrict__ sub_bits, szk_layout_params lp, int do_layout) {
+    if (do_layout && blockIdx.x == 0 && threadIdx.x == 0) layout_pre(lp);
     const bool seg_ok = *seg_made != 0;
     const uint64_t n_vec = (n_segs + 7) / 8;
     const uint64_t n_vec16 = (n_vec + 15) / 16 * 16;
@@ -3696,7 +3726,7 @@
     return (total_bits + 31) >> 5;
 }
 
-__device__ void assemble_body(const szk_asm_params &p, uint64_t tid, uint64_t nth) {
+__device__ void assemble_body(const szk_asm_params &p, uint64_t tid, uint64_t nth, const uint64_t *total_in = nullptr) {
     __shared__ szh_header s_h0, s_h;
     __shared__ szh_offsets s_o, s_oo;
     if (threadIdx.x == 0) {
@@ -3710,7 +3740,7 @@
         szh_header &h = s_h;
         szh_offsets &oo = s_oo;
         h = s_h0;
-        h.bitstream_words = *p.total_words;
+        h.bitstream_words = total_in ? *total_in : *p.total_words;
         szh_compute_offsets(h, oo);
         h.payload_bytes = oo.end;
         *reinterpret_cast<szh_header *>(p.payload) = h;
@@ -4065,6 +4095,7 @@
 #define PB_THREADS 1024u
 #define PB_WAVES (PB_THREADS / WAVE)
 #define PB_ASM_BLOCKS 32u
+#define PB_SCAN_GROUPS 4096u
 __device__ __forceinline__ void packb_emit(uint64_t *stage, uint64_t val, uint32_t len, uint32_t pos) {
     const uint64_t v = val << ((64u - len) & 63u);
     const uint32_t q = pos >> 6, sh = pos & 63u;
@@ -4157,8 +4188,13 @@
 __global__ __launch_bounds__(PB_THREADS) void k_pack_b(const uint16_t *__restrict__ codes, uint64_t n, const uint32_t *__restrict__ g_enc,
                                                         const uint16_t *__restrict__ chunk_words, const uint64_t *__restrict__ group_off, szk_mode mode,
                                                         uint32_t sym_add, const szk_state *__restrict__ state, uint8_t *__restrict__ payload,
-                                                        szk_asm_params ap, uint32_t pack_blocks, uint32_t split, szk_role_params rp, uint32_t only_sampled) {
+                                                        szk_asm_params ap, uint32_t pack_blocks, uint32_t split, szk_role_params rp, uint32_t only_sampled,
+                                                        const uint32_t *__restrict__ group_sums) {
     constexpr int STAGE_WORDS = SZH_CHUNK_SYMS * SZH_MAX_LEN / 32 + 4;
+    static_assert(PB_SCAN_GROUPS == 4u * PB_THREADS, "four groups per thread");
+    __shared__ __align__(16) uint32_t s_goff[PB_SCAN_GROUPS];
+    __shared__ uint32_t s_scan_w[PB_WAVES];
+    __shared__ uint64_t s_total;
     __shared__ __align__(16) uint32_t s_pair[128 * 128];
     __shared__ uint32_t s_enc8[256];
     __shared__ uint8_t s_plen8[256];
@@ -4173,7 +4209,21 @@
     const uint32_t asm_blocks = gridDim.x - roles - pack_blocks;
     if (blockIdx.x >= roles + pack_blocks) {
         const uint32_t ab = blockIdx.x - roles - pack_blocks;
-        assemble_body(ap, (uint64_t)ab * PB_THREADS + threadIdx.x, (uint64_t)asm_blocks * PB_THREADS);
+        if (group_sums && ab == 0) {
+            const uint64_t n_groups = ((n + SZH_CHUNK_SYMS - 1) / SZH_CHUNK_SYMS + PACK_GROUP - 1) / PACK_GROUP;
+            uint32_t mine = 0;
+            for (uint64_t g = threadIdx.x; g < n_groups; g += PB_THREADS) mine += group_sums[g];
+            mine = wave_sum(mine);
+            if (lane_id() == 0) s_scan_w[threadIdx.x / WAVE] = mine;
+            __syncthreads();
+            if (threadIdx.x == 0) {
+                uint64_t tot = 0;
+                for (uint32_t w = 0; w < PB_WAVES; w++) tot += s_scan_w[w];
+                s_total = tot;
+            }
+            __syncthreads();
+        }
+        assemble_body(ap, (uint64_t)ab * PB_THREADS + threadIdx.x, (uint64_t)asm_blocks * PB_THREADS, group_sums ? &s_total : nullptr);
         if (!ap.lists_by_roles) assemble_lists(ap, (uint64_t)ab * PB_THREADS + threadIdx.x, (uint64_t)asm_blocks * PB_THREADS);
         return;
     }
@@ -4210,7 +4260,22 @@
 #pragma unroll
         for (uint32_t j = 0; j < PB_BATCH; j++) cur[j] = fetch(unit * PB_BATCH + j);
         fr_cur = front_of(unit);
-        go_cur = group_off[unit * PB_BATCH / PACK_GROUP];
+        if (!group_sums) go_cur = group_off[unit * PB_BATCH / PACK_GROUP];
+    }
+    uint32_t gsum[4] = {0u, 0u, 0u, 0u}, gmine = 0, gincl = 0;
+    if (group_sums) {
+        const uint64_t n_groups = (n_chunks + PACK_GROUP - 1) / PACK_GROUP;
+        const uint32_t g0 = 4u * threadIdx.x;
+        if (g0 < n_groups) {
+            const uint4 q = *reinterpret_cast<const uint4 *>(group_sums + g0);
+            gsum[0] = q.x;
+            gsum[1] = g0 + 1 < n_groups ? q.y : 0u;
+            gsum[2] = g0 + 2 < n_groups ? q.z : 0u;
+            gsum[3] = g0 + 3 < n_groups ? q.w : 0u;
+        }
+        gmine = gsum[0] + gsum[1] + gsum[2] + gsum[3];
+        gincl = wave_incl_scan(gmine);
+        if (lane == WAVE - 1) s_scan_w[wv] = gincl;
     }
     if (threadIdx.x < 256u) {
         const uint32_t e = g_enc[threadIdx.x != 255u ? threadIdx.x + sym_add : 0u];
@@ -4219,6 +4284,15 @@
     }
     for (int i = lane; i < STAGE_WORDS / 2; i += WAVE) stage[i] = 0;
     __syncthreads();
+    if (group_sums) {
+        uint32_t run = gincl - gmine;
+        for (uint32_t w = 0; w < wv; w++) run += s_scan_w[w];
+#pragma unroll
+        for (int j = 0; j < 4; j++) {
+            s_goff[4u * threadIdx.x + j] = run;
+            run += gsum[j];
+        }
+    }
     for (uint32_t i = threadIdx.x; i < 128u * 128u; i += PB_THREADS) {
         const uint32_t i1 = i >> 7, i0 = (i & 127u) ^ i1;
         const uint32_t t0 = i0 < 64u ? i0 + 128u : i0, t1 = i1 < 64u ? i1 + 128u : i1;
@@ -4227,13 +4301,14 @@
         s_pair[i] = (l0 && l1 && len <= 27u) ? ((((s_enc8[t0] << l1) | s_enc8[t1]) << 5) | len) : 0u;
     }
     __syncthreads();
+    if (group_sums && unit < n_units) go_cur = s_goff[unit * PB_BATCH / PACK_GROUP];
     for (; unit < n_units; unit += nwaves) {
         const uint64_t nu = unit + nwaves;
         if (nu < n_units) {
 #pragma unroll
             for (uint32_t j = 0; j < PB_BATCH; j++) nxt[j] = fetch(nu * PB_BATCH + j);
             fr_nxt = front_of(nu);
-            go_nxt = group_off[nu * PB_BATCH / PACK_GROUP];
+            go_nxt = group_sums ? (uint64_t)s_goff[nu * PB_BATCH / PACK_GROUP] : group_off[nu * PB_BATCH / PACK_GROUP];
         }
         uint32_t *out = out_base + go_cur + wave_sum(fr_cur);
         const uint64_t c_lo = unit * PB_BATCH;
@@ -4243,12 +4318,21 @@
                 const uint32_t nwords = packb_chunk(cur[j], s_pair, s_enc8, s_plen8, stage);
                 __builtin_amdgcn_fence(__ATOMIC_RELEASE, "workgroup");
                 __builtin_amdgcn_wave_barrier();
-                for (uint32_t i = 2 * lane; i < nwords + 2; i += 2 * WAVE) {
-                    const uint64_t v = stage[i >> 1];
-                    stage[i >> 1] = 0;
-                    if (lab_nost && v != 0x123456789abcdefull) continue;
-                    if (i < nwords) out[i] = __builtin_bswap32((uint32_t)(v >> 32));
-                    if (i + 1 < nwords) out[i + 1] = __builtin_bswap32((uint32_t)v);
+                for (uint32_t i0 = 2 * lane; i0 < nwords + 2; i0 += 4 * WAVE) {
+#pragma unroll
+                    for (uint32_t h = 0; h < 2; h++) {
+                        const uint32_t i = i0 + h * 2 * WAVE;
+                        if (i < nwords + 2) {
+                            const uint64_t v = stage[i >> 1];
+                            stage[i >> 1] = 0;
+                            if (lab_nost && v != 0x123456789abcdefull) continue;
+                            const uint32_t w0 = __builtin_bswap32((uint32_t)(v >> 32)), w1 = __builtin_bswap32((uint32_t)v);
+                            if (i + 1 < nwords) {
+                                struct __attribute__((packed, aligned(4))) pair32 { uint64_t v; };
+                                reinterpret_cast<pair32 *>(out + i)->v = (uint64_t)w0 | ((uint64_t)w1 << 32);
+                            } else if (i < nwords) out[i] = w0;
+                        }
+                    }
                 }
                 __builtin_amdgcn_wave_barrier();
                 out += nwords;
@@ -4289,7 +4373,7 @@
         const uint32_t before = wave_sum(bp);
         __builtin_amdgcn_fence(__ATOMIC_RELEASE, "workgroup");
         __builtin_amdgcn_wave_barrier();
-        uint32_t *out = out_base + group_off[grp] + before;
+        uint32_t *out = out_base + (group_sums ? (uint64_t)s_goff[grp] : group_off[grp]) + before;
         for (uint32_t i = lane; i < nwords; i += WAVE) out[i] = __builtin_bswap32((uint32_t)(stage[i >> 1] >> ((i & 1u) ? 0 : 32)));
     }
 }
@@ -5841,6 +5925,11 @@
     SZK_CHECK_LAUNCH();
     return 0;
 }
+bool szk_encode_scans_in_packer(uint64_t n, const szk_asm_params *asmp, bool seg, const szk_encode_roles *er) {
+    const uint64_t n_chunks = (n + SZH_CHUNK_SYMS - 1) / SZH_CHUNK_SYMS, n_groups = (n_chunks + PACK_GROUP - 1) / PACK_GROUP;
+    return seg && asmp && er && er->roles && er->no_book && !er->fold_rows && asmp->samp_words && asmp->assumed_narrow && n_chunks >= 4096 &&
+           n_groups <= PB_SCAN_GROUPS;
+}
 int szk_launch_encode(const uint16_t *codes, uint64_t n, const uint32_t *d_enc, const szk_cb_info *info, int radius,
                       szk_mode mode, uint16_t *chunk_words, uint64_t *group_off, uint64_t *total_words,
                       const szk_state *state, uint8_t *payload, const szk_layout_params *layout, const szk_asm_params *asmp, hipStream_t s,
@@ -5861,15 +5950,19 @@
         fp.range = er->fold_range;
     }
     const uint16_t *scan_in = nullptr;
+    const bool pack_scan = !mg && szk_encode_scans_in_packer(n, asmp, seg_bits != nullptr, er);
+    const uint32_t *pack_sums = nullptr;
     if (seg_bits) {
         const uint64_t n_segs = (n + 255) / 256;
-        uint32_t *gsums = reinterpret_cast<uint32_t *>(group_off + (n_chunks + PACK_GROUP - 1) / PACK_GROUP + 1);
+        uint32_t *gsums = pack_scan ? reinterpret_cast<uint32_t *>(group_off) : reinterpret_cast<uint32_t *>(group_off + (n_chunks + PACK_GROUP - 1) / PACK_GROUP + 1);
         hipLaunchKernelGGL(k_seg_chunks, dim3((uint32_t)std::min<uint64_t>(((n_segs + 7) / 8 + 255) / 256, 1024)), dim3(256), 0, s, seg_bits, n_segs, seg_made,
-                           chunk_words, n_chunks, gsums, sub_bits);
+                           chunk_words, n_chunks, gsums, sub_bits, *layout, pack_scan ? 1 : 0);
         scan_in = reinterpret_cast<const uint16_t *>(gsums);
-    }
-    hipLaunchKernelGGL(k_scan_groups, dim3(fp.nrows ? 65 : 1), dim3(1024), 0, s, chunk_words, n_chunks, group_off, total_words, *layout, 1, scan_in,
-                       (uint64_t)0, seg_made, fp);
+        if (pack_scan) pack_sums = gsums;
+    }
+    if (!pack_scan)
+        hipLaunchKernelGGL(k_scan_groups, dim3(fp.nrows ? 65 : 1), dim3(1024), 0, s, chunk_words, n_chunks, group_off, total_words, *layout, 1, scan_in,
+                           (uint64_t)0, seg_made, fp);
     szk_role_params rp{};
     szk_asm_params apv = asmp ? *asmp : szk_asm_params{};
     if (er && er->roles && asmp) {
@@ -5916,7 +6009,7 @@
         beside |= (szk_dbg_flags & 512) ? 16u : 0u;
 #endif
         hipLaunchKernelGGL(k_pack_b, dim3(rb + PB_ASM_BLOCKS + pb), dim3(PB_THREADS), 0, s, codes, n, d_enc, chunk_words, group_off, mode, sym_add, state,
-                           payload, apv, pb, split, rp, beside);
+                           payload, apv, pb, split, rp, beside, pack_sums);
         if (beside & 1u) {
             const uint32_t pb2 = pgrid < 1280 - extra ? pgrid : 1280 - extra;
             hipLaunchKernelGGL((k_pack<ENC_WIN>), dim3(rb + pb2 + (asmp ? ASM_BLOCKS : 0)), dim3(256), 0, s, codes, n, d_enc, info, chunk_words, group_off, mode,
```

Result: slower. 2256 GB/s (-1.0%).
